# eridgd/WCT-TF

Measured on AMD Instinct MI355X. Metric: stylized frames/sec @512x512, 5-level relu5->1 pipeline, alpha=0.8, higher is better.
Workload: dtype f16

## Files before the change

### wct_tf_amd/csrc/api.hip

```cpp
#include "common.h"
#include "../../include/wct_hip.h"

#include <stdarg.h>
#include <stdio.h>
#include <string.h>
#include <stdlib.h>
#include <vector>
#include <cmath>
#include <algorithm>

static thread_local char g_err[512] = "";
void wct_set_error(const char* fmt, ...) {
  va_list ap;
  va_start(ap, fmt);
  vsnprintf(g_err, sizeof(g_err), fmt, ap);
  va_end(ap);
}
extern "C" const char* wct_last_error(void) { return g_err; }

struct DevBuf {
  void* p = nullptr;
  size_t cap = 0;
};

// ... 370 lines not shown
extern "C" int wct_set_encoder(wct_ctx* c, const float* pre_w, const float* pre_b,
                               const float* const* w, const float* const* b, int n_layers) {
  ARG_CHECK(c && pre_w && pre_b && w && b && n_layers == 13);
  HIP_TRY(hipSetDevice(c->device));
  std::vector<float> fw(27 * 64), fb(64);
  const float* w1 = w[0];
  for (int co = 0; co < 64; ++co) {
    double acc = b[0][co];
    for (int tap = 0; tap < 9; ++tap)
      for (int cp = 0; cp < 3; ++cp) acc += (double)pre_b[cp] * w1[(tap * 3 + cp) * 64 + co];
    fb[co] = (float)acc;
  }
  for (int tap = 0; tap < 9; ++tap)
    for (int ci = 0; ci < 3; ++ci)
      for (int co = 0; co < 64; ++co) {
        double acc = 0;
        for (int cp = 0; cp < 3; ++cp) acc += (double)pre_w[ci * 3 + cp] * w1[(tap * 3 + cp) * 64 + co];
        fw[(tap * 3 + ci) * 64 + co] = (float)acc;
      }
  if (c->first_w) { hipFree(c->first_w); c->first_w = nullptr; }
  if (c->first_b) { hipFree(c->first_b); c->first_b = nullptr; }
  std::vector<half_t> frag(2 * 2 * 2 * 64 * 8);
  for (int t = 0; t < 2; ++t)
    for (int ks = 0; ks < 2; ++ks)
      for (int l = 0; l < 64; ++l)
        for (int j = 0; j < 8; ++j) {
          const int co = t * 32 + (l & 31), k = ks * 16 + (l >> 5) * 8 + j;
          const float wv = k < 27 ? fw[k * 64 + co] : 0.f;
          const half_t hi = (half_t)wv;
          const half_t lo = (half_t)(wv - (float)hi);
          frag[((((t * 2 + ks) * 2 + 0) * 64) + l) * 8 + j] = hi;
          frag[((((t * 2 + ks) * 2 + 1) * 64) + l) * 8 + j] = lo;
        }
  TRY(upload(c, frag.data(), frag.size() * sizeof(half_t), (void**)&c->first_w));
  TRY(upload(c, fb.data(), fb.size() * sizeof(float), (void**)&c->first_b));
  if (c->first_w32) { hipFree(c->first_w32); c->first_w32 = nullptr; }
  TRY(upload(c, fw.data(), fw.size() * sizeof(float), (void**)&c->first_w32));
  for (int i = 0; i < 12; ++i) {
    TRY(pack_conv(c, w[i + 1], b[i + 1], ENC_CIN[i], ENC_COUT[i], &c->enc[i]));
    const int cin = ENC_CIN[i], cout = ENC_COUT[i];
    std::vector<float> wt((size_t)9 * cin * cout);
    for (int tap = 0; tap < 9; ++tap)
      for (int ci = 0; ci < cin; ++ci)
        for (int co = 0; co < cout; ++co) wt[((size_t)tap * cout + co) * cin + ci] = w[i + 1][((size_t)tap * cin + ci) * cout + co];
    if (c->enc_wt[i]) { hipFree(c->enc_wt[i]); c->enc_wt[i] = nullptr; }
    TRY(upload(c, wt.data(), wt.size() * sizeof(float), (void**)&c->enc_wt[i]));
  }
  c->enc_loaded = true;
  return WCT_OK;
}

static std::vector<PlanStep> decoder_plan(int level) {
  static const int arch5[] = {512, -1, 512, 512, 512, 0};
  static const int arch4[] = {256, -1, 256, 256, 256, 0};
  static const int arch3[] = {128, -1, 128, 0};
  static const int arch2[] = {64, -1, 0};
  static const int arch1[] = {64, 0};
  static const int* archs[6] = {nullptr, arch1, arch2, arch3, arch4, arch5};
  std::vector<PlanStep> plan;
  int cin = LEVEL_C[level];
  for (int d = level; d >= 1; --d)
    for (const int* a = archs[d]; *a != 0; ++a) {
      if (*a < 0) plan.push_back({'U', cin, cin, 0});
      else { plan.push_back({'C', cin, *a, 1}); cin = *a; }
    }
  plan.push_back({'C', cin, 3, 0});
  return plan;
}

extern "C" int wct_set_decoder(wct_ctx* c, int level, const float* const* w, const float* const* b, int n_layers) {
  ARG_CHECK(c && w && b && level >= 1 && level <= 5);
  HIP_TRY(hipSetDevice(c->device));
  Decoder& d = c->dec[level];
  free_decoder(d);
  d.plan = decoder_plan(level);
  int nconv = 0;
  for (auto& s : d.plan) nconv += s.kind == 'C';
  if (n_layers != nconv) {
    wct_set_error("decoder relu%d_1 needs %d conv layers, got %d", level, nconv, n_layers);
    return WCT_ERR_ARG;
  }
  int i = 0;
  for (auto& s : d.plan) {
    if (s.kind != 'C') continue;
    if (s.cout == 3) {
      std::vector<half_t> w16((size_t)4 * 64 * 8);
      for (int ks = 0; ks < 4; ++ks)
        for (int l = 0; l < 64; ++l)
          for (int j = 0; j < 8; ++j) {
            const int row = l & 31, cin = ks * 16 + (l >> 5) * 8 + j;
            const int tap = row / 3, co = row % 3;
            w16[((size_t)ks * 64 + l) * 8 + j] = row < 27 ? (half_t)w[i][((size_t)tap * 64 + cin) * 3 + co] : (half_t)0.f;
          }
      TRY(upload(c, w16.data(), w16.size() * sizeof(half_t), (void**)&d.last_w));
      TRY(upload(c, b[i], 3 * sizeof(float), (void**)&d.last_b));
    } else {
      d.convs.emplace_back();
      TRY(pack_conv(c, w[i], b[i], s.cin, s.cout, &d.convs.back()));
    }
    {
      float *w32 = nullptr, *b32 = nullptr;
      TRY(upload(c, w[i], (size_t)9 * s.cin * s.cout * sizeof(float), (void**)&w32));
      TRY(upload(c, b[i], (size_t)s.cout * sizeof(float), (void**)&b32));
      d.w32.push_back(w32); d.b32.push_back(b32); d.cin.push_back(s.cin); d.cout.push_back(s.cout);
    }
    ++i;
  }
  d.loaded = true;
  return WCT_OK;
}

static void level_dims(int H, int W, int level, int* h, int* w) {
  for (int l = 1; l < level; ++l) { H = (H + 1) / 2; W = (W + 1) / 2; }
  *h = H; *w = W;
}

static int check_min_size(const char* what, int H, int W, int level) {
  int h, w;
  level_dims(H, W, level, &h, &w);
  if (h < 2 || w < 2) {
    wct_set_error("%s %dx%d is too small for relu%d_1: its %dx%d feature map cannot be reflect-padded (need >= %dx%d pixels)",
                  what, H, W, level, h, w, (1 << (level - 1)) + 1, (1 << (level - 1)) + 1);
    return WCT_ERR_ARG;
  }
  return WCT_OK;
}


static int run_conv(wct_ctx* c, const ConvLayer& l, const half_t* x, half_t* y16, float* y32,
                    int B, int H, int W, int upsample, int relu, int pool = 0, float* usum = nullptr, unsigned* umax = nullptr,
                    bool tap_layer = false) {
  ConvArgs a;
  a.x = x; a.w = l.w; a.bias = l.b; a.y16 = y16; a.y32 = y32; a.usum = usum; a.umax = umax;
  a.w_wino = c->no_wino || tap_layer ? nullptr : l.ww;
  a.B = B; a.H = H; a.W = W; a.Cin = l.cin; a.Cout = l.cout; a.upsample = upsample; a.relu = relu; a.pool = pool;
  const double px = (double)B * H * W;
  const double in_px = upsample ? px / 4 : px;
  const double out_px = pool ? (double)B * ((H + 1) / 2) * ((W + 1) / 2) : px;
  ProfScope ps(c, conv3x3_wino_takes(a) ? 9 : 0, 2.0 * px * 9 * l.cin * l.cout,
               in_px * l.cin * 2 + out_px * l.cout * ((y16 ? 2 : 0) + (y32 ? 4 : 0)) + 9.0 * l.cin * l.cout * 2);
  return launch_conv3x3(a, c->stream);
}

static int run_encoder(wct_ctx* c, const float* img, int B, int H, int W, int clamp01, int deepest,
                       float* const taps32[6], float* const* usum = nullptr, unsigned* const* umax = nullptr) {
  if (!c->enc_loaded) { wct_set_error("encoder weights not set (wct_set_encoder)"); return WCT_ERR_STATE; }
  ARG_CHECK(deepest >= 1 && deepest <= 5 && H >= 2 && W >= 2);
  const size_t act_bytes = (size_t)B * H * W * 64 * sizeof(half_t);
  TRY(ensure(c, c->act[0], act_bytes));
  TRY(ensure(c, c->act[1], act_bytes));
  half_t* cur = (half_t*)c->act[0].p;
  half_t* nxt = (half_t*)c->act[1].p;
  static const int fuse_conv1_env = getenv("WCT_FUSE_CONV1") ? atoi(getenv("WCT_FUSE_CONV1")) : 1;
  const bool fuse_conv1 = fuse_conv1_env && deepest > 1 && !taps32[1];
  if (!fuse_conv1) {
    ConvFirstArgs a;
    a.x = img; a.wfrag = c->first_w; a.bias = c->first_b;
    a.y16 = deepest > 1 ? cur : nullptr; a.y32 = taps32[1];
    a.B = B; a.H = H; a.W = W; a.clamp01 = clamp01;
    a.usum = usum && taps32[1] ? usum[1] : nullptr; a.umax = a.usum ? umax[1] : nullptr;
    const double px = (double)B * H * W;
    ProfScope ps(c, 1, 2.0 * px * 27 * 64, px * (12 + 64 * ((a.y16 ? 2 : 0) + (a.y32 ? 4 : 0))));
    TRY(launch_conv_first(a, c->stream));
  }
  if (deepest == 1) return WCT_OK;
  static const int seq_tap[12] = {0, 2, 0, 3, 0, 0, 0, 4, 0, 0, 0, 5};
  static const int pool_after[12] = {1, 0, 1, 0, 0, 0, 1, 0, 0, 0, 1, 0};
  int h = H, w = W;
  for (int i = 0; i < 12; ++i) {
    const ConvLayer& l = c->enc[i];
    const int tap = seq_tap[i];
    const bool last = tap == deepest;
    const bool fuse = pool_after[i];
    float* const us = tap && taps32[tap] && usum ? usum[tap] : nullptr;
    if (i == 0 && fuse_conv1) {
      ConvArgs a;
      a.x = nullptr; a.w = l.w; a.bias = l.b; a.y16 = nxt; a.y32 = nullptr; a.usum = nullptr; a.umax = nullptr;
      a.B = B; a.H = h; a.W = w; a.Cin = 64; a.Cout = 64; a.upsample = 0; a.relu = 1; a.pool = fuse;
      a.img1 = img; a.w1frag = c->first_w; a.bias1 = c->first_b; a.clamp01 = clamp01;
      const double px = (double)B * h * w, out_px = fuse ? (double)B * ((h + 1) / 2) * ((w + 1) / 2) : px;
      ProfScope ps(c, 8, 2.0 * px * (27 * 64 + 9 * 64 * 64), px * 12 + out_px * 64 * 2 + 9.0 * 64 * 64 * 2);
      TRY(launch_conv3x3(a, c->stream));
    } else
    TRY(run_conv(c, l, cur, last ? nullptr : nxt, tap ? taps32[tap] : nullptr, B, h, w, 0, 1, fuse, us, us ? umax[tap] : nullptr, tap != 0));
    half_t* t = cur; cur = nxt; nxt = t;
    if (last) break;
    if (fuse) { h = (h + 1) / 2; w = (w + 1) / 2; }
  }
  return WCT_OK;
}

static int run_decoder(wct_ctx* c, int level, const half_t* feat16, int B, int h, int w, float* img_out) {
  Decoder& d = c->dec[level];
  if (!d.loaded) { wct_set_error("decoder weights for relu%d_1 not set (wct_set_decoder)", level); return WCT_ERR_STATE; }
  const int scale = 1 << (level - 1);
  const size_t act_bytes = (size_t)B * h * scale * w * scale * 64 * sizeof(half_t);
  const size_t deep_bytes = (size_t)B * h * w * LEVEL_C[level] * sizeof(half_t) * 4;
  TRY(ensure(c, c->act[0], act_bytes > deep_bytes ? act_bytes : deep_bytes));
  TRY(ensure(c, c->act[1], act_bytes > deep_bytes ? act_bytes : deep_bytes));
  const half_t* cur = feat16;
  half_t* bufs[2] = {(half_t*)c->act[0].p, (half_t*)c->act[1].p};
  int which = 0, ci = 0, up = 0;
  const size_t nsteps = d.plan.size();
  for (size_t si = 0; si < nsteps; ++si) {
    const PlanStep& s = d.plan[si];
    if (s.kind == 'U') { up = 1; h *= 2; w *= 2; continue; }
    if (s.cout == 3) {
      ARG_CHECK(up == 0);
      ConvLastArgs a;
      a.x = cur; a.wfrag = d.last_w; a.bias = d.last_b; a.y = img_out; a.B = B; a.H = h; a.W = w;
      const double px = (double)B * h * w;
      ProfScope ps(c, 2, 2.0 * px * 576 * 3, px * (128 + 12));
      TRY(launch_conv_last(a, c->stream));
    } else {
      half_t* out = bufs[which];
      TRY(run_conv(c, d.convs[ci++], cur, out, nullptr, B, h, w, up, 1));
      cur = out; which ^= 1; up = 0;
    }
  }
  return WCT_OK;
}

struct StageCost { double cov_flops, cov_bytes, apply_flops, apply_bytes, adain_bytes; };

template <typename Launch>
static int run_stages(wct_ctx* c, size_t ws_bytes, unsigned flags, const StageCost& cost, Launch&& launch) {
  TRY(ensure(c, c->wct_ws, ws_bytes));
  if (flags & WCT_FLAG_ADAIN) {
    ProfScope ps(c, 7, 0, cost.adain_bytes);
    return launch(0, 0);
  }
  const int mode = (flags & WCT_FLAG_MODE_NP) ? WCT_MODE_NP : WCT_MODE_TF;
  {
    ProfScope ps(c, 4, cost.cov_flops, cost.cov_bytes);
    TRY(launch(mode, WCT_STAGE_COV));
  }
  {
    ProfScope ps(c, 5, 0, 0);
    TRY(launch(mode, WCT_STAGE_EIG));
  }
  ProfScope ps(c, 6, cost.apply_flops, cost.apply_bytes);
  return launch(mode, WCT_STAGE_APPLY);
}

static int run_transform(wct_ctx* c, const float* fc, int Nc, const float* fs, int Ns, int C, int P,
                         float alpha, unsigned flags, float eps, half_t* out16, float* out32, int* sweeps_dev,
                         const WctFeatStats* st = nullptr, const WctStyleRef* prep = nullptr ,
                         const WctWarmRef* warm = nullptr ) {
  const int shared = (flags & WCT_FLAG_STYLE_SHARED) ? 1 : 0;
  const StageCost cost = {(double)P * 2.0 * C * C * ((double)Nc + Ns), (double)P * 2.0 * ((double)Nc + Ns) * C * 4,
                          (double)P * (2.0 * C * C * Nc + 6.0 * C * C * C), (double)P * Nc * C * (4 + (out16 ? 2 : 0) + (out32 ? 4 : 0)),
                          (double)P * (2.0 * Nc + 2.0 * Ns) * C * 4 + (double)P * Nc * C * 6};
  return run_stages(c, wct_workspace_bytes(C, Nc, Ns, P), flags, cost, [&](int mode, int stages) {
    if (!stages) return launch_adain(fc, Nc, fs, Ns, C, P, alpha, 1e-5f, out16, out32, c->wct_ws.p, c->wct_ws.cap, c->stream, shared, st, prep);
    return launch_wct(fc, Nc, fs, Ns, C, P, alpha, mode, eps, out16, out32, c->wct_ws.p, c->wct_ws.cap, sweeps_dev, stages, c->stream,
                      shared, c->eig_fail_dev, st, prep, warm);
  });
}

static int mix_weights(const float* weights, int K, float* lambda) {
  if (K < 1 || K > WCT_MIX_MAX) { wct_set_error("style mix: K = %d styles, must be 1 .. %d", K, (int)WCT_MIX_MAX); return WCT_ERR_ARG; }
  if (!weights) { wct_set_error("style mix: no weights"); return WCT_ERR_ARG; }
  double sum = 0.0;
  for (int k = 0; k < K; ++k) {
    if (!(weights[k] >= 0.f) || !std::isfinite(weights[k])) {
      wct_set_error("style mix: weight %d is %g; weights must be finite and >= 0", k, (double)weights[k]);
      return WCT_ERR_ARG;
    }
    sum += weights[k];
  }
  if (!(sum > 0.0) || !std::isfinite(sum)) { wct_set_error("style mix: the weights sum to %g, must be > 0", sum); return WCT_ERR_ARG; }
  for (int k = 0; k < K; ++k) lambda[k] = (float)(weights[k] / sum);
  return WCT_OK;
}

static int run_transform_mix(wct_ctx* c, const float* fc, int Nc, const float* const* fs, const int* Ns, int K, const float* lambda,
                             int C, float alpha, unsigned flags, float eps, half_t* out16, float* out32, int* sweeps_dev,
                             const WctFeatStats* st = nullptr, const WctStyleRef* prep = nullptr ) {
  double ns = 0;
  for (int k = 0; k < K; ++k) ns += Ns[k];
  const StageCost cost = {2.0 * C * C * (Nc + ns), 2.0 * (Nc + ns) * C * 4, 2.0 * C * C * Nc + 6.0 * C * C * C * (K + 1) + 2.0 * C * C * K,
                          (double)Nc * C * (4 + (out16 ? 2 : 0) + (out32 ? 4 : 0)), (2.0 * Nc + 2.0 * ns) * C * 4 + (double)Nc * C * 6};
  return run_stages(c, wct_mix_workspace_bytes(C, Nc, Ns, K, lambda), flags, cost, [&](int mode, int stages) {
    if (!stages) return launch_adain_mix(fc, Nc, fs, Ns, K, lambda, C, alpha, 1e-5f, out16, out32, c->wct_ws.p, c->wct_ws.cap, c->stream, st, prep);
    return launch_wct_mix(fc, Nc, fs, Ns, K, lambda, C, alpha, mode, eps, out16, out32, c->wct_ws.p, c->wct_ws.cap, sweeps_dev, stages,
                          c->stream, c->eig_fail_dev, st, prep);
  });
}

static int mask_check(const uint8_t* labels, size_t n, int K) {
  if (K < 1 || K > WCT_MIX_MAX) { wct_set_error("mask: K = %d styles, must be 1 .. %d", K, (int)WCT_MIX_MAX); return WCT_ERR_ARG; }
  uint8_t top = 0;
  for (size_t i = 0; i < n; ++i) top = labels[i] > top ? labels[i] : top;
  if (top >= K) { wct_set_error("mask: label %d with K = %d styles (labels must be 0 .. K - 1)", (int)top, K); return WCT_ERR_ARG; }
  return WCT_OK;
}

static void mask_counts(const uint8_t* mask, int Hm, int Wm, int h, int w, int stride, int K, int* nk) {
  for (int k = 0; k < K; ++k) nk[k] = 0;
  for (int i = 0; i < h; ++i) {
    const uint8_t* row = mask + (size_t)std::min(i * stride, Hm - 1) * Wm;
    for (int j = 0; j < w; ++j) ++nk[row[std::min(j * stride, Wm - 1)]];
  }
}

static int run_transform_masked(wct_ctx* c, const float* fc, int Nc, const MaskGeom& g, const int* nk, const float* const* fs,
                                const int* Ns, int K, int C, float alpha, unsigned flags, float eps, half_t* out16, float* out32,
                                int* sweeps_dev) {
  double ns = 0;
  int P = 0;
  for (int k = 0; k < K; ++k) { ns += nk[k] >= 2 ? Ns[k] : 0; P += nk[k] >= 2; }
  const StageCost cost = {2.0 * C * C * (Nc + ns), (4.0 * Nc + 2.0 * (Nc + ns)) * C * 4, 2.0 * C * C * Nc + 6.0 * C * C * C * P,
                          (double)Nc * C * (4 + (out16 ? 2 : 0) + (out32 ? 4 : 0)), (4.0 * Nc + 2.0 * ns) * C * 4 + (double)Nc * C * 6};
  return run_stages(c, wct_masked_workspace_bytes(C, Nc, nk, Ns, K), flags, cost, [&](int mode, int stages) {
    if (!stages) return launch_adain_masked(fc, Nc, g, nk, fs, Ns, K, C, alpha, 1e-5f, out16, out32, c->wct_ws.p, c->wct_ws.cap, c->stream);
    return launch_wct_masked(fc, Nc, g, nk, fs, Ns, K, C, alpha, mode, eps, out16, out32, c->wct_ws.p, c->wct_ws.cap, sweeps_dev, stages,
                             c->stream, c->eig_fail_dev);
  });
}

static int stage_in(wct_ctx* c, int slot, const void* host, size_t bytes, void** dev) {
  TRY(ensure(c, c->stage[slot], bytes));
  HIP_TRY(hipMemcpyAsync(c->stage[slot].p, host, bytes, hipMemcpyHostToDevice, c->stream));
  *dev = c->stage[slot].p;
  return WCT_OK;
}
static int fetch(wct_ctx* c, void* host, const void* dev, size_t bytes) {
  HIP_TRY(hipMemcpyAsync(host, dev, bytes, hipMemcpyDeviceToHost, c->stream));
  HIP_TRY(hipStreamSynchronize(c->stream));
  return WCT_OK;
}

extern "C" int wct_transform(wct_ctx* c, const float* content, int Nc, const float* style, int Ns, int C,
                             float alpha, int mode, float eps, float* out, int* sweeps_out) {
  ARG_CHECK(c && content && style && out && (mode == WCT_NP || mode == WCT_TF));
  HIP_TRY(hipSetDevice(c->device));
  TRY(eig_stale(c));
  void *dc, *ds;
  TRY(stage_in(c, 0, content, (size_t)Nc * C * 4, &dc));
  TRY(stage_in(c, 1, style, (size_t)Ns * C * 4, &ds));
  TRY(ensure(c, c->stage[2], (size_t)Nc * C * 4));
  TRY(ensure(c, c->stage[3], 256));
  TRY(run_transform(c, (float*)dc, Nc, (float*)ds, Ns, C, 1, alpha, mode == WCT_NP ? WCT_FLAG_MODE_NP : 0, eps,
                    nullptr, (float*)c->stage[2].p, (int*)c->stage[3].p));
  TRY(fetch(c, out, c->stage[2].p, (size_t)Nc * C * 4));
  if (sweeps_out) TRY(fetch(c, sweeps_out, c->stage[3].p, 2 * sizeof(int)));
  return eig_status(c);
}

extern "C" int wct_adain(wct_ctx* c, const float* content, int Nc, const float* style, int Ns, int C,
                         float alpha, float epsilon, float* out) {
  ARG_CHECK(c && content && style && out);
  HIP_TRY(hipSetDevice(c->device));
  void *dc, *ds;
  TRY(stage_in(c, 0, content, (size_t)Nc * C * 4, &dc));
  TRY(stage_in(c, 1, style, (size_t)Ns * C * 4, &ds));
  TRY(ensure(c, c->stage[2], (size_t)Nc * C * 4));
  TRY(ensure(c, c->wct_ws, wct_workspace_bytes(C, Nc, Ns, 1)));
  TRY(launch_adain((float*)dc, Nc, (float*)ds, Ns, C, 1, alpha, epsilon, nullptr, (float*)c->stage[2].p,
                   c->wct_ws.p, c->wct_ws.cap, c->stream, 0));
  return fetch(c, out, c->stage[2].p, (size_t)Nc * C * 4);
}

static int stage_in_multi(wct_ctx* c, const float* content, int Nc, const float* const* styles, const int* Ns, int K, int C,
                          void** dc, const float* ds[]) {
  TRY(stage_in(c, 0, content, (size_t)Nc * C * 4, dc));
  size_t total = 0;
  for (int k = 0; k < K; ++k) { ARG_CHECK(styles[k] && Ns[k] >= 1); total += (size_t)Ns[k] * C * 4; }
  TRY(ensure(c, c->mix_in, total));
  size_t off = 0;
  for (int k = 0; k < K; ++k) {
    char* d = (char*)c->mix_in.p + off;
    HIP_TRY(hipMemcpyAsync(d, styles[k], (size_t)Ns[k] * C * 4, hipMemcpyHostToDevice, c->stream));
    ds[k] = (const float*)d;
    off += (size_t)Ns[k] * C * 4;
  }
  TRY(ensure(c, c->stage[2], (size_t)Nc * C * 4));
  return ensure(c, c->stage[3], 2 * WCT_MIX_MAX * sizeof(int));
}

extern "C" int wct_transform_mix(wct_ctx* c, const float* content, int Nc, const float* const* styles, const int* Ns, int K,
                                 const float* weights, int C, float alpha, int mode, float eps, float* out, int* sweeps_out) {
  ARG_CHECK(c && content && styles && Ns && out && (mode == WCT_NP || mode == WCT_TF));
  float lambda[WCT_MIX_MAX];
  TRY(mix_weights(weights, K, lambda));
  HIP_TRY(hipSetDevice(c->device));
  TRY(eig_stale(c));
  void* dc;
  const float* ds[WCT_MIX_MAX];
  TRY(stage_in_multi(c, content, Nc, styles, Ns, K, C, &dc, ds));
  TRY(run_transform_mix(c, (float*)dc, Nc, ds, Ns, K, lambda, C, alpha, mode == WCT_NP ? WCT_FLAG_MODE_NP : 0, eps,
                        nullptr, (float*)c->stage[2].p, (int*)c->stage[3].p));
  TRY(fetch(c, out, c->stage[2].p, (size_t)Nc * C * 4));
  if (sweeps_out) {
    int sw[2 * WCT_MIX_MAX];
    TRY(fetch(c, sw, c->stage[3].p, 2 * K * sizeof(int)));
    sweeps_out[0] = sw[0];
    for (int k = 0; k < K; ++k) sweeps_out[1 + k] = sw[2 * k + 1];
  }
  return eig_status(c);
}

extern "C" int wct_adain_mix(wct_ctx* c, const float* content, int Nc, const float* const* styles, const int* Ns, int K,
                             const float* weights, int C, float alpha, float epsilon, float* out) {
// ... 242 lines not shown
  TRY(ensure(c, c->stage[1], (size_t)H * W * C * 2));
  TRY(ensure(c, c->stage[2], (size_t)Ho * Wo * C * 2));
  TRY(ensure(c, c->stage[3], (size_t)Ho * Wo * C * 4));
  TRY(launch_f32_to_f16((float*)dx, (half_t*)c->stage[1].p, (size_t)H * W * C, c->stream));
  TRY(launch_maxpool2x2((half_t*)c->stage[1].p, (half_t*)c->stage[2].p, 1, H, W, C, c->stream));
  TRY(launch_f16_to_f32((half_t*)c->stage[2].p, (float*)c->stage[3].p, (size_t)Ho * Wo * C, c->stream));
  return fetch(c, y, c->stage[3].p, (size_t)Ho * Wo * C * 4);
}

extern "C" int wct_encode(wct_ctx* c, const float* img01, int H, int W, int level, float* feat) {
  ARG_CHECK(c && img01 && feat && level >= 1 && level <= 5);
  HIP_TRY(hipSetDevice(c->device));
  TRY(check_min_size("image", H, W, level));
  int h, w;
  level_dims(H, W, level, &h, &w);
  void* dimg;
  TRY(stage_in(c, 0, img01, (size_t)H * W * 3 * 4, &dimg));
  const size_t fb = (size_t)h * w * LEVEL_C[level] * 4;
  TRY(ensure(c, c->feat_c, fb));
  float* taps[6] = {nullptr, nullptr, nullptr, nullptr, nullptr, nullptr};
  taps[level] = (float*)c->feat_c.p;
  TRY(run_encoder(c, (float*)dimg, 1, H, W, 0, level, taps));
  return fetch(c, feat, c->feat_c.p, fb);
}

extern "C" int wct_decode(wct_ctx* c, const float* feat, int h, int w, int level, float* img) {
  ARG_CHECK(c && feat && img && level >= 1 && level <= 5);
  HIP_TRY(hipSetDevice(c->device));
  const int C = LEVEL_C[level], scale = 1 << (level - 1);
  void* df;
  TRY(stage_in(c, 0, feat, (size_t)h * w * C * 4, &df));
  TRY(ensure(c, c->wct_out, (size_t)h * w * C * 2));
  TRY(launch_f32_to_f16((float*)df, (half_t*)c->wct_out.p, (size_t)h * w * C, c->stream));
  const size_t ib = (size_t)h * scale * w * scale * 3 * 4;
  TRY(ensure(c, c->img_t[0], ib));
  TRY(run_decoder(c, level, (half_t*)c->wct_out.p, 1, h, w, (float*)c->img_t[0].p));
  return fetch(c, img, c->img_t[0].p, ib);
}

extern "C" int wct_coral_stats(wct_ctx* c, const uint8_t* img, int H, int W, double sums[9]) {
  ARG_CHECK(c && img && sums && H > 0 && W > 0);
  HIP_TRY(hipSetDevice(c->device));
  const size_t npix = (size_t)H * W;
  void* dimg;
  TRY(stage_in(c, 0, img, npix * 3, &dimg));
  int nblocks = (int)((npix + 255) / 256);
  if (nblocks > 1024) nblocks = 1024;
  TRY(ensure(c, c->stage[1], (size_t)(nblocks + 1) * 9 * sizeof(unsigned long long)));
  unsigned long long* partial = (unsigned long long*)c->stage[1].p;
  unsigned long long* out9 = partial + (size_t)nblocks * 9;
  TRY(launch_coral_stats((uint8_t*)dimg, npix, partial, nblocks, out9, c->stream));
  unsigned long long host9[9];
  TRY(fetch(c, host9, out9, sizeof(host9)));
  for (int k = 0; k < 9; ++k) sums[k] = (double)host9[k];
  return WCT_OK;
}

extern "C" int wct_coral_apply(wct_ctx* c, const uint8_t* src, int H, int W, const double M[9],
                               const double src_mean[3], const double src_std[3], const double tgt_mean[3],
                               const double tgt_std[3], uint8_t* out_u8, double* out_f64) {
  ARG_CHECK(c && src && M && src_mean && src_std && tgt_mean && tgt_std && (out_u8 || out_f64) && H > 0 && W > 0);
  HIP_TRY(hipSetDevice(c->device));
  const size_t npix = (size_t)H * W;
  CoralApplyArgs a;
  for (int i = 0; i < 9; ++i) a.M[i] = M[i];
  for (int i = 0; i < 3; ++i) { a.src_mean[i] = src_mean[i]; a.src_std[i] = src_std[i]; a.tgt_mean[i] = tgt_mean[i]; a.tgt_std[i] = tgt_std[i]; }
  void* dsrc;
  TRY(stage_in(c, 0, src, npix * 3, &dsrc));
  if (out_u8) TRY(ensure(c, c->stage[1], npix * 3));
  if (out_f64) TRY(ensure(c, c->stage[2], npix * 3 * sizeof(double)));
  TRY(launch_coral_apply((uint8_t*)dsrc, npix, a, out_u8 ? (uint8_t*)c->stage[1].p : nullptr,
                         out_f64 ? (double*)c->stage[2].p : nullptr, c->stream));
  if (out_u8) TRY(fetch(c, out_u8, c->stage[1].p, npix * 3));
  if (out_f64) TRY(fetch(c, out_f64, c->stage[2].p, npix * 3 * sizeof(double)));
  return WCT_OK;
}

static int content_colors_checks(const void* stylized, int Ho, int Wo, const void* content, int Hc, int Wc, int B, const void* out) {
  if (!stylized || !content || !out) { wct_set_error("content colours: null image pointer"); return WCT_ERR_ARG; }
  if (B < 1 || B > 32) { wct_set_error("content colours: B = %d frames, must be 1 .. 32", B); return WCT_ERR_ARG; }
  if (Hc < 1 || Wc < 1 || Ho < Hc || Wo < Wc) {
    wct_set_error("content colours: a %dx%d stylized frame for a %dx%d content (the frame is never the smaller one)", Ho, Wo, Hc, Wc);
    return WCT_ERR_ARG;
  }
  return WCT_OK;
}

extern "C" int wct_content_colors_batch_dev(wct_ctx* c, const uint8_t* stylized, int Ho, int Wo, const uint8_t* content, int Hc,
                                            int Wc, int B, uint8_t* out) {
  ARG_CHECK(c != nullptr);
  TRY(content_colors_checks(stylized, Ho, Wo, content, Hc, Wc, B, out));
  HIP_TRY(hipSetDevice(c->device));
  ProfScope ps(c, 7, 0, (double)B * Ho * Wo * 3 * 2 + (double)B * Hc * Wc * 3);
  return launch_content_colors_u8(stylized, content, B, Ho, Wo, Hc, Wc, out, c->stream);
}

extern "C" int wct_content_colors(wct_ctx* c, const uint8_t* stylized, int Ho, int Wo, const uint8_t* content, int Hc, int Wc,
                                  uint8_t* out) {
  ARG_CHECK(c != nullptr);
  TRY(content_colors_checks(stylized, Ho, Wo, content, Hc, Wc, 1, out));
  HIP_TRY(hipSetDevice(c->device));
  void *ds, *dc;
  TRY(stage_in(c, 0, stylized, (size_t)Ho * Wo * 3, &ds));
  TRY(stage_in(c, 1, content, (size_t)Hc * Wc * 3, &dc));
  TRY(wct_content_colors_batch_dev(c, (uint8_t*)ds, Ho, Wo, (uint8_t*)dc, Hc, Wc, 1, (uint8_t*)ds));
  return fetch(c, out, ds, (size_t)Ho * Wo * 3);
}

extern "C" int wct_output_size(int Hc, int Wc, const int* levels, int n_levels, int* Ho, int* Wo) {
  ARG_CHECK(levels && Ho && Wo && n_levels >= 1 && Hc >= 2 && Wc >= 2);
  int H = Hc, W = Wc;
  for (int i = 0; i < n_levels; ++i) {
    ARG_CHECK(levels[i] >= 1 && levels[i] <= 5);
    TRY(check_min_size("content", H, W, levels[i]));
    int h, w;
    level_dims(H, W, levels[i], &h, &w);
    H = h << (levels[i] - 1); W = w << (levels[i] - 1);
  }
  *Ho = H; *Wo = W;
  return WCT_OK;
}

static int stylize_checks(wct_ctx* c, int Hc, int Wc, const uint8_t* const* styles, const int* Hs, const int* Ws, int K,
                          const int* levels, int n_levels, int* deepest, int* Ho, int* Wo) {
  *deepest = 0;
  for (int i = 0; i < n_levels; ++i) {
    ARG_CHECK(levels[i] >= 1 && levels[i] <= 5);
    if (levels[i] > *deepest) *deepest = levels[i];
    if (!c->dec[levels[i]].loaded) { wct_set_error("decoder weights for relu%d_1 not set", levels[i]); return WCT_ERR_STATE; }
  }
  TRY(wct_output_size(Hc, Wc, levels, n_levels, Ho, Wo));
  for (int k = 0; k < K; ++k) { ARG_CHECK(styles[k]); TRY(check_min_size("style", Hs[k], Ws[k], *deepest)); }
  return WCT_OK;
}

static int images_f32(wct_ctx* c, unsigned flags, const void* content, size_t nc, const void* style, size_t ns, const float** img_c,
                      const float** img_s) {
  *img_c = (const float*)content; *img_s = (const float*)style;
  if (flags & WCT_FLAG_IMAGES_F32) return WCT_OK;
  TRY(ensure(c, c->img_c, nc * 4));
  TRY(ensure(c, c->img_s, ns * 4));
  ProfScope ps(c, 7, 0, (double)(nc + ns) * 5);
  TRY(launch_u8_to_f32((const uint8_t*)content, (float*)c->img_c.p, nc, c->stream));
  TRY(launch_u8_to_f32((const uint8_t*)style, (float*)c->img_s.p, ns, c->stream));
  *img_c = (const float*)c->img_c.p; *img_s = (const float*)c->img_s.p;
  return WCT_OK;
}

static bool fuse_stats() {
  static const int on = getenv("WCT_FUSE_STATS") ? atoi(getenv("WCT_FUSE_STATS")) : 1;
  return on != 0;
}

template <typename StyleAt, typename Transform>
static int stylize_levels(wct_ctx* c, const float* img_c, const void* content_raw, int B, int Hc, int Wc, const int* levels,
                          int n_levels, unsigned flags, size_t umax_clear, int clear_from, StyleAt&& style_at,
                          Transform&& transform, uint8_t* out) {
  unsigned* const umax_c = (unsigned*)c->umax.p;
  const float* cur = img_c;
  int H = Hc, W = Wc;
  for (int i = 0; i < n_levels; ++i) {
    const int l = levels[i], C = LEVEL_C[l];
    int h, w;
    level_dims(H, W, l, &h, &w);
    TRY(ensure(c, c->feat_c, (size_t)B * h * w * C * 4));
    float* ctaps[6] = {nullptr, nullptr, nullptr, nullptr, nullptr, nullptr};
    ctaps[l] = (float*)c->feat_c.p;
    float* us_c[6] = {nullptr, nullptr, nullptr, nullptr, nullptr, nullptr};
    unsigned* um_c[6] = {nullptr, nullptr, nullptr, nullptr, nullptr, nullptr};
    if (fuse_stats() && w % 16 == 0) {
      TRY(ensure(c, c->usum_c, (size_t)B * h * (w / 16) * C * 4));
      us_c[l] = (float*)c->usum_c.p; um_c[l] = umax_c;
      if (i >= clear_from) HIP_TRY(hipMemsetAsync(umax_c, 0, umax_clear, c->stream));
    }
    WctFeatStats st = {};
    st.u[0] = us_c[l]; st.umax[0] = um_c[l];
    TRY(run_encoder(c, cur, B, H, W, i > 0, l, ctaps, us_c, um_c));
    TRY(ensure(c, c->wct_out, (size_t)B * h * w * C * 2));
    if (l == 5 && (flags & WCT_FLAG_SWAP5)) {
      int hs, ws;
      style_at(l, 0, &hs, &ws);
      ARG_CHECK(h >= c->ss_patch && w >= c->ss_patch && hs >= c->ss_patch && ws >= c->ss_patch);
      TRY(ensure(c, c->wct_ws, style_swap_workspace_bytes(C, h, w, hs, ws, c->ss_patch, c->ss_stride)));
      ProfScope ps(c, 7, 0, 0);
      for (int b = 0; b < B; ++b)
        TRY(launch_style_swap((float*)c->feat_c.p + (size_t)b * h * w * C, h, w, style_at(l, b, &hs, &ws), hs, ws, C, c->ss_alpha,
                              c->ss_patch, c->ss_stride, -1.f, (half_t*)c->wct_out.p + (size_t)b * h * w * C, nullptr,
                              c->wct_ws.p, c->wct_ws.cap, c->stream, c->eig_fail_dev));
    } else
      TRY(transform(i, l, C, h, w, st));
    const int scale = 1 << (l - 1);
    const int H2 = h * scale, W2 = w * scale;
    DevBuf& dst = c->img_t[i & 1];
    TRY(ensure(c, dst, (size_t)B * H2 * W2 * 3 * 4));
    TRY(run_decoder(c, l, (half_t*)c->wct_out.p, B, h, w, (float*)dst.p));
    cur = (float*)dst.p; H = H2; W = W2;
  }
  if (flags & WCT_FLAG_CONTENT_COLORS) {
    const int f32 = (flags & WCT_FLAG_IMAGES_F32) ? 1 : 0;
    ProfScope ps(c, 7, 0, (double)B * H * W * 3 * 5 + (double)B * Hc * Wc * 3 * (f32 ? 4 : 1));
    return launch_content_colors_f32(cur, content_raw, f32, B, H, W, Hc, Wc, out, c->stream);
  }
  ProfScope ps(c, 7, 0, (double)B * H * W * 3 * 5);
  return launch_f32_to_u8(cur, out, (size_t)B * H * W * 3, c->stream);
}

extern "C" int wct_stylize_batch_dev(wct_ctx* c, const uint8_t* content, int Hc, int Wc, const uint8_t* style,
                                     int Hs, int Ws, int B, const int* levels, int n_levels, float alpha,
                                     unsigned flags, uint8_t* out) {
  ARG_CHECK(c && content && style && out && levels && n_levels >= 1 && n_levels <= 16 && B >= 1 && B <= 32);
  HIP_TRY(hipSetDevice(c->device));
  int deepest, Ho, Wo;
  TRY(stylize_checks(c, Hc, Wc, &style, &Hs, &Ws, 1, levels, n_levels, &deepest, &Ho, &Wo));

  const int shared = (flags & WCT_FLAG_STYLE_SHARED) ? 1 : 0;
  const int Bs = shared ? 1 : B;
  const float *img_c, *img_s;
  TRY(images_f32(c, flags, content, (size_t)B * Hc * Wc * 3, style, (size_t)Bs * Hs * Ws * 3, &img_c, &img_s));
  const bool want_stats = fuse_stats();
  constexpr size_t UROW = 32 * UMAX_SLOTS;
  TRY(ensure(c, c->umax, 7 * UROW * sizeof(unsigned)));
  unsigned* const umax_c = (unsigned*)c->umax.p;
  if (want_stats) HIP_TRY(hipMemsetAsync(c->umax.p, 0, 7 * UROW * sizeof(unsigned), c->stream));
  float* taps[6] = {nullptr, nullptr, nullptr, nullptr, nullptr, nullptr};
  float* us_s[6] = {nullptr, nullptr, nullptr, nullptr, nullptr, nullptr};
  unsigned* um_s[6] = {nullptr, nullptr, nullptr, nullptr, nullptr, nullptr};
  for (int i = 0; i < n_levels; ++i) {
    const int l = levels[i];
    int h, w;
    level_dims(Hs, Ws, l, &h, &w);
    TRY(ensure(c, c->feat_s[l], (size_t)Bs * h * w * LEVEL_C[l] * 4));
    taps[l] = (float*)c->feat_s[l].p;
    if (want_stats && w % 16 == 0) {
      TRY(ensure(c, c->usum_s[l], (size_t)Bs * h * (w / 16) * LEVEL_C[l] * 4));
      us_s[l] = (float*)c->usum_s[l].p; um_s[l] = umax_c + UROW * l;
    }
  }
  TRY(run_encoder(c, img_s, Bs, Hs, Ws, 0, deepest, taps, us_s, um_s));

  auto style_at = [&](int l, int b, int* hs, int* ws) {
    level_dims(Hs, Ws, l, hs, ws);
    return (const float*)c->feat_s[l].p + (size_t)(shared ? 0 : b) * *hs * *ws * LEVEL_C[l];
  };
  return stylize_levels(c, img_c, content, B, Hc, Wc, levels, n_levels, flags, UROW * sizeof(unsigned), 1, style_at,
                        [&](int, int l, int C, int h, int w, WctFeatStats st) {
                          int hs, ws;
                          const float* fs = style_at(l, 0, &hs, &ws);
                          st.u[1] = us_s[l]; st.umax[1] = um_s[l];
                          return run_transform(c, (float*)c->feat_c.p, h * w, fs, hs * ws, C, B, alpha, flags, -1.f,
                                               (half_t*)c->wct_out.p, nullptr, nullptr, &st);
                        }, out);
}

extern "C" int wct_stylize(wct_ctx* c, const uint8_t* content, int Hc, int Wc, const uint8_t* style, int Hs, int Ws,
                           const int* levels, int n_levels, float alpha, unsigned flags, uint8_t* out) {
  ARG_CHECK(c && content && style && out);
  HIP_TRY(hipSetDevice(c->device));
  TRY(eig_stale(c));
  int Ho, Wo;
  TRY(wct_output_size(Hc, Wc, levels, n_levels, &Ho, &Wo));
  void *dc, *ds;
  const size_t px = (flags & WCT_FLAG_IMAGES_F32) ? sizeof(float) : 1;
  TRY(stage_in(c, 0, content, (size_t)Hc * Wc * 3 * px, &dc));
  TRY(stage_in(c, 1, style, (size_t)Hs * Ws * 3 * px, &ds));
  TRY(ensure(c, c->stage[2], (size_t)Ho * Wo * 3));
  TRY(wct_stylize_batch_dev(c, (uint8_t*)dc, Hc, Wc, (uint8_t*)ds, Hs, Ws, 1, levels, n_levels, alpha, flags,
                            (uint8_t*)c->stage[2].p));
  TRY(fetch(c, out, c->stage[2].p, (size_t)Ho * Wo * 3));
  return eig_status(c);
}

template <typename LevelTransform>
static int stylize_multi(wct_ctx* c, const uint8_t* content, int Hc, int Wc, const uint8_t* const* styles, const int* Hs,
                         const int* Ws, int K, const int* levels, int n_levels, unsigned flags, uint8_t* out,
                         LevelTransform&& level_transform) {
  HIP_TRY(hipSetDevice(c->device));
  int deepest, Ho, Wo;
  TRY(stylize_checks(c, Hc, Wc, styles, Hs, Ws, K, levels, n_levels, &deepest, &Ho, &Wo));
  TRY(eig_stale(c));
  const size_t px = (flags & WCT_FLAG_IMAGES_F32) ? sizeof(float) : 1;
  size_t ns_tot = 0, soff[WCT_MIX_MAX];
  for (int k = 0; k < K; ++k) { soff[k] = ns_tot; ns_tot += (size_t)Hs[k] * Ws[k] * 3; }
  const size_t nc = (size_t)Hc * Wc * 3;
  void* dc;
  TRY(stage_in(c, 0, content, nc * px, &dc));
  TRY(ensure(c, c->mix_in, ns_tot * px));
  for (int k = 0; k < K; ++k)
    HIP_TRY(hipMemcpyAsync((char*)c->mix_in.p + soff[k] * px, styles[k], (size_t)Hs[k] * Ws[k] * 3 * px, hipMemcpyHostToDevice, c->stream));
  const float *img_c, *img_s;
  TRY(images_f32(c, flags, dc, nc, c->mix_in.p, ns_tot, &img_c, &img_s));

  size_t foff[6][WCT_MIX_MAX];
  for (int i = 0; i < n_levels; ++i) {
    const int l = levels[i];
    size_t tot = 0;
    for (int k = 0; k < K; ++k) {
      int h, w;
      level_dims(Hs[k], Ws[k], l, &h, &w);
      foff[l][k] = tot;
      tot += (size_t)h * w * LEVEL_C[l];
    }
    TRY(ensure(c, c->feat_mix[l], tot * 4));
  }
  for (int k = 0; k < K; ++k) {
    float* taps[6] = {nullptr, nullptr, nullptr, nullptr, nullptr, nullptr};
    for (int i = 0; i < n_levels; ++i) taps[levels[i]] = (float*)c->feat_mix[levels[i]].p + foff[levels[i]][k];
    TRY(run_encoder(c, img_s + soff[k], 1, Hs[k], Ws[k], 0, deepest, taps));
  }

  TRY(ensure(c, c->umax, 32 * UMAX_SLOTS * sizeof(unsigned)));
  TRY(ensure(c, c->stage[2], (size_t)Ho * Wo * 3));
  auto style_at = [&](int l, int k, int* hs, int* ws) {
    level_dims(Hs[k], Ws[k], l, hs, ws);
    return (const float*)c->feat_mix[l].p + foff[l][k];
  };
  TRY(stylize_levels(c, img_c, dc, 1, Hc, Wc, levels, n_levels, flags, UMAX_SLOTS * sizeof(unsigned), 0, style_at,
                     [&](int i, int l, int C, int h, int w, const WctFeatStats& st) {
                       const float* fs[WCT_MIX_MAX];
                       int Ns[WCT_MIX_MAX];
                       for (int k = 0; k < K; ++k) {
                         int hs, ws;
                         fs[k] = style_at(l, k, &hs, &ws);
                         Ns[k] = hs * ws;
                       }
                       return level_transform(i, l, C, h, w, fs, Ns, &st);
                     }, (uint8_t*)c->stage[2].p));
  TRY(fetch(c, out, c->stage[2].p, (size_t)Ho * Wo * 3));
  return eig_status(c);
}

extern "C" int wct_stylize_mix(wct_ctx* c, const uint8_t* content, int Hc, int Wc, const uint8_t* const* styles, const int* Hs,
                               const int* Ws, int K, const float* weights, const int* levels, int n_levels, float alpha,
                               unsigned flags, uint8_t* out) {
  ARG_CHECK(c && content && styles && Hs && Ws && out && levels && n_levels >= 1 && n_levels <= 16);
  float lambda[WCT_MIX_MAX];
  TRY(mix_weights(weights, K, lambda));
  if ((flags & WCT_FLAG_SWAP5) && K > 1) {
    wct_set_error("style mix: WCT_FLAG_SWAP5 needs K = 1 (style-swap is not linear in the style; got K = %d)", K);
    return WCT_ERR_ARG;
  }
  if (flags & WCT_FLAG_STYLE_SHARED) { wct_set_error("style mix: WCT_FLAG_STYLE_SHARED is for wct_stylize_batch_dev"); return WCT_ERR_ARG; }
  return stylize_multi(c, content, Hc, Wc, styles, Hs, Ws, K, levels, n_levels, flags, out,
                       [&](int, int, int C, int h, int w, const float* const* fs, const int* Ns, const WctFeatStats* st) {
                         return run_transform_mix(c, (float*)c->feat_c.p, h * w, fs, Ns, K, lambda, C, alpha, flags, -1.f,
                                                  (half_t*)c->wct_out.p, nullptr, nullptr, st);
                       });
}

extern "C" int wct_stylize_masked(wct_ctx* c, const uint8_t* content, int Hc, int Wc, const uint8_t* mask, const uint8_t* const* styles,
                                  const int* Hs, const int* Ws, int K, const int* levels, int n_levels, float alpha, unsigned flags,
                                  uint8_t* out) {
  ARG_CHECK(c && content && mask && styles && Hs && Ws && out && levels && n_levels >= 1 && n_levels <= 16 && Hc >= 2 && Wc >= 2);
  TRY(mask_check(mask, (size_t)Hc * Wc, K));
  if ((flags & WCT_FLAG_SWAP5) && K > 1) {
    wct_set_error("mask: WCT_FLAG_SWAP5 needs K = 1 (style-swap is not a per-region affine map; got K = %d)", K);
    return WCT_ERR_ARG;
  }
  if (flags & WCT_FLAG_STYLE_SHARED) { wct_set_error("mask: WCT_FLAG_STYLE_SHARED is for wct_stylize_batch_dev"); return WCT_ERR_ARG; }
  std::vector<int> nk((size_t)n_levels * WCT_MIX_MAX);
  int H = Hc, W = Wc;
  for (int i = 0; i < n_levels; ++i) {
    ARG_CHECK(levels[i] >= 1 && levels[i] <= 5);
    int h, w;
    level_dims(H, W, levels[i], &h, &w);
    mask_counts(mask, Hc, Wc, h, w, 1 << (levels[i] - 1), K, &nk[(size_t)i * WCT_MIX_MAX]);
    H = h << (levels[i] - 1); W = w << (levels[i] - 1);
  }
  HIP_TRY(hipSetDevice(c->device));
  TRY(ensure(c, c->mask_in, (size_t)Hc * Wc));
  HIP_TRY(hipMemcpyAsync(c->mask_in.p, mask, (size_t)Hc * Wc, hipMemcpyHostToDevice, c->stream));
  return stylize_multi(c, content, Hc, Wc, styles, Hs, Ws, K, levels, n_levels, flags, out,
                       [&](int i, int l, int C, int h, int w, const float* const* fs, const int* Ns, const WctFeatStats*) {
                         const MaskGeom g = {(const uint8_t*)c->mask_in.p, Hc, Wc, w, 1 << (l - 1)};
                         return run_transform_masked(c, (float*)c->feat_c.p, h * w, g, &nk[(size_t)i * WCT_MIX_MAX], fs, Ns, K, C,
                                                     alpha, flags, -1.f, (half_t*)c->wct_out.p, nullptr, nullptr);
                       });
}

static int style_live(const wct_ctx* c, const wct_style* st) {
  if (st && std::find(c->styles.begin(), c->styles.end(), st) != c->styles.end()) return WCT_OK;
  wct_set_error("prepared style %p is not a live handle of this context (freed, or prepared by another context)", (const void*)st);
  return WCT_ERR_STATE;
}

static StyleState* state_find(wct_style* st, int level, const WctStyleKey& key, int kind) {
  for (auto& e : st->cache[level])
    if (e.kind == kind && e.key.nslab == key.nslab && e.key.nsplit == key.nsplit && e.key.ksplit == key.ksplit) return &e;
  return nullptr;
}

struct StyleNeed { int level; WctStyleKey key; int kind; };

static int style_fill(wct_ctx* c, wct_style* st, const std::vector<StyleNeed>& needs) {
  if (needs.empty()) return WCT_OK;
  HIP_TRY(hipStreamSynchronize(c->stream));
  int deepest = 0;
  float* taps[6] = {nullptr, nullptr, nullptr, nullptr, nullptr, nullptr};
  for (const StyleNeed& n : needs) {
    int h, w;
    level_dims(st->Hs, st->Ws, n.level, &h, &w);
    TRY(ensure(c, c->feat_s[n.level], (size_t)h * w * LEVEL_C[n.level] * 4));
    taps[n.level] = (float*)c->feat_s[n.level].p;
    deepest = std::max(deepest, n.level);
  }
// ... 760 lines not shown
```

### wct_tf_amd/csrc/common.h

```cpp
#pragma once
#include <hip/hip_runtime.h>
#include <stdint.h>
#include <stddef.h>

typedef _Float16 half_t;
typedef _Float16 half8 __attribute__((ext_vector_type(8)));
typedef _Float16 half4 __attribute__((ext_vector_type(4)));
typedef float f32x16 __attribute__((ext_vector_type(16)));
typedef float f32x4 __attribute__((ext_vector_type(4)));

#define WCT_OK 0
#define WCT_ERR_HIP -1
#define WCT_ERR_ARG -2
#define WCT_ERR_STATE -3
#define WCT_ERR_NOMEM -4
#define WCT_ERR_NOCONV -5

void wct_set_error(const char* fmt, ...);

#define HIP_TRY(expr)                                                          \
  do {                                                                         \
    hipError_t _e = (expr);                                                    \
    if (_e != hipSuccess) {                                                    \
      wct_set_error("%s failed: %s (%s:%d)", #expr, hipGetErrorString(_e),     \
                    __FILE__, __LINE__);                                       \
      return WCT_ERR_HIP;                                                      \
    }                                                                          \
  } while (0)

#define ARG_CHECK(cond)                                                        \
  do {                                                                         \
    if (!(cond)) {                                                             \
      wct_set_error("invalid argument: %s (%s:%d)", #cond, __FILE__, __LINE__);\
      return WCT_ERR_ARG;                                                      \
    }                                                                          \
  } while (0)

static inline int cdiv(int a, int b) { return (a + b - 1) / b; }


struct ConvArgs {
  const half_t* x;
  const half_t* w;
  const float* bias;
  half_t* y16;
  float* y32;
  int B, H, W;
  int Cin, Cout;
  int upsample;
  int relu;
  int pool;
  float* usum;
  unsigned* umax;
  const float* img1 = nullptr;
  const half_t* w1frag = nullptr;
  const float* bias1 = nullptr;
  int clamp01 = 0;
  const half_t* w_wino = nullptr;
};
constexpr int UMAX_SLOTS = 64;
__device__ __forceinline__ void umax_merge(unsigned* umax_img, int slot, float vmax, int lane) {
#pragma unroll
  for (int o = 32; o > 0; o >>= 1) vmax = fmaxf(vmax, __shfl_xor(vmax, o, 64));
  if (lane == 0) {
    unsigned* w = umax_img + (slot & (UMAX_SLOTS - 1));
    const unsigned bits = __builtin_bit_cast(unsigned, vmax);
    if (bits > __atomic_load_n(w, __ATOMIC_RELAXED)) atomicMax(w, bits);
  }
}
int launch_conv3x3(const ConvArgs& a, hipStream_t s);
bool conv3x3_wino_takes(const ConvArgs& a);
int launch_conv3x3_wino(const ConvArgs& a, hipStream_t s);

struct ConvFirstArgs {
  const float* x;
  const half_t* wfrag;
  const float* bias;
  half_t* y16;
  float* y32;
  int B, H, W;
  int clamp01;
  float* usum;
  unsigned* umax;
};

__device__ __forceinline__ void unit_row_sum4(f32x4& t) {
  float a = t[0], b = t[1], c = t[2], d = t[3];
#define WCT_DPP_STEP(ctrl)                                                             \
  "v_add_f32_dpp %0, %0, %0 " ctrl " row_mask:0xf bank_mask:0xf bound_ctrl:1\n"       \
  "v_add_f32_dpp %1, %1, %1 " ctrl " row_mask:0xf bank_mask:0xf bound_ctrl:1\n"       \
  "v_add_f32_dpp %2, %2, %2 " ctrl " row_mask:0xf bank_mask:0xf bound_ctrl:1\n"       \
  "v_add_f32_dpp %3, %3, %3 " ctrl " row_mask:0xf bank_mask:0xf bound_ctrl:1\n"
  asm volatile("s_nop 1\n"
               WCT_DPP_STEP("quad_perm:[1,0,3,2]")
               WCT_DPP_STEP("quad_perm:[2,3,0,1]")
               WCT_DPP_STEP("row_half_mirror")
               WCT_DPP_STEP("row_mirror")
               : "+v"(a), "+v"(b), "+v"(c), "+v"(d));
#undef WCT_DPP_STEP
  t[0] = a; t[1] = b; t[2] = c; t[3] = d;
}
int launch_conv_first(const ConvFirstArgs& a, hipStream_t s);

struct ConvLastArgs {
  const half_t* x;
  const half_t* wfrag;
  const float* bias;
  float* y;
  int B, H, W;
};
int launch_conv_last(const ConvLastArgs& a, hipStream_t s);

int launch_maxpool2x2(const half_t* x, half_t* y, int B, int H, int W, int C, hipStream_t s);
int launch_u8_to_f32(const uint8_t* x, float* y, size_t n, hipStream_t s);
int launch_f32_to_u8(const float* x, uint8_t* y, size_t n, hipStream_t s);
int launch_f32_to_f16(const float* x, half_t* y, size_t n, hipStream_t s);
int launch_f16_to_f32(const half_t* x, float* y, size_t n, hipStream_t s);

struct GemmArgs {
  const float* A; int lda; int a_kmajor;
  const float* B; int ldb; int b_kmajor;
  const float* a_sub_m;
  const float* b_sub_n;
  const float* a_sub_k;
  const float* a_scale_k;
  int M, N, K;
  int ksplit;
  float* out32; half_t* out16; int ldo;
  size_t out_split_stride;
  const float* bias_n;
  int nsplit;
  size_t sA, sB, s_sub_m, s_sub_n, s_sub_k, s_scale_k, s_out, s_bias;
  const float* A_odd;
  size_t sA_odd;
  int skip_shared;
  int blend; float alpha; unsigned* mabs;
  const float* mask_diag; size_t s_mask; int* mask_out; const int* mask_in;
};

int launch_gemm(GemmArgs g, int nsplit, int nbatch, hipStream_t s);

enum { WCT_MODE_NP = 0, WCT_MODE_TF = 1 };

struct WctFeatStats { const float* u[2]; const unsigned* umax[2]; };

struct WctStyleKey { int nslab, nsplit, ksplit; };
WctStyleKey wct_style_key(int C, int Nc, int Ns);
size_t wct_style_state_floats(int C);
size_t wct_style_workspace_bytes(int C, int Ns, const WctStyleKey& key);
int launch_style_state(const float* style, int Ns, int C, const WctStyleKey& key, int adain, int mode, float eps, void* workspace,
                       size_t workspace_bytes, int* eig_fail, hipStream_t s, float* state);
struct WctStyleRef { const float* state[8]; };
struct WctStyleSlots { const float* state[32]; };

struct WctWarmRef { float* basis; int valid; };

size_t wct_workspace_bytes(int C, int Nc, int Ns, int P);
int launch_wct(const float* content, int Nc, const float* style, int Ns, int C, int P,
               float alpha, int mode, float eps , half_t* out16, float* out32,
               void* workspace, size_t workspace_bytes, int* sweeps_dev, int stages, hipStream_t s,
               int shared_style ,
               int* eig_fail ,
               const struct WctFeatStats* stats = nullptr ,
               const struct WctStyleRef* prep = nullptr ,
               const struct WctWarmRef* warm = nullptr );
enum { WCT_STAGE_COV = 1, WCT_STAGE_EIG = 2, WCT_STAGE_APPLY = 4, WCT_STAGE_ALL = 7, WCT_STAGE_EIG_FP32UPDATE = 8 };
int launch_adain(const float* content, int Nc, const float* style, int Ns, int C, int P,
                 float alpha, float eps, half_t* out16, float* out32,
                 void* workspace, size_t workspace_bytes, hipStream_t s, int shared_style,
                 const struct WctFeatStats* stats = nullptr, const struct WctStyleRef* prep = nullptr);
enum { WCT_MIX_MAX = 8 };
size_t wct_mix_workspace_bytes(int C, int Nc, const int* Ns, int K, const float* lambda);
int launch_wct_mix(const float* content, int Nc, const float* const* styles, const int* Ns, int K, const float* lambda, int C,
                   float alpha, int mode, float eps, half_t* out16, float* out32, void* workspace, size_t workspace_bytes,
                   int* sweeps_dev, int stages, hipStream_t s, int* eig_fail, const struct WctFeatStats* stats = nullptr,
                   const struct WctStyleRef* prep = nullptr);
int launch_adain_mix(const float* content, int Nc, const float* const* styles, const int* Ns, int K, const float* lambda, int C,
                     float alpha, float eps, half_t* out16, float* out32, void* workspace, size_t workspace_bytes, hipStream_t s,
                     const struct WctFeatStats* stats = nullptr, const struct WctStyleRef* prep = nullptr);
struct MaskGeom { const uint8_t* mask; int Hm, Wm, w, stride; };
size_t mask_compact_workspace_bytes(int N, int G = 1);
int launch_mask_compact(const MaskGeom& g, int N, int K, int* perm, int* seg_off, void* workspace, hipStream_t s);
size_t wct_masked_workspace_bytes(int C, int Nc, const int* nk, const int* Ns, int K);
int launch_wct_masked(const float* content, int Nc, const MaskGeom& g, const int* nk, const float* const* styles, const int* Ns, int K,
                      int C, float alpha, int mode, float eps, half_t* out16, float* out32, void* workspace, size_t workspace_bytes,
                      int* sweeps_dev, int stages, hipStream_t s, int* eig_fail);
int launch_adain_masked(const float* content, int Nc, const MaskGeom& g, const int* nk, const float* const* styles, const int* Ns, int K,
                        int C, float alpha, float eps, half_t* out16, float* out32, void* workspace, size_t workspace_bytes, hipStream_t s);
size_t wct_masked_batch_workspace_bytes(int C, int Nc, int G, const int* nk, const int* Ns, int K);
int wct_masked_batch_pairs(int G, const int* nk, int K);
int launch_mask_compact_batch(const MaskGeom& g, int N, int K, int G, int* perm, int* seg_off, void* workspace, hipStream_t s);
int launch_wct_masked_batch(const float* content, int Nc, int G, const MaskGeom& g, const int* nk, const int* Ns, int K,
                            const WctStyleSlots& states, int C, float alpha, int mode, float eps, half_t* out16, float* out32,
                            void* workspace, size_t workspace_bytes, int stages, hipStream_t s, int* eig_fail);
int launch_adain_masked_batch(const float* content, int Nc, int G, const MaskGeom& g, const int* nk, const int* Ns, int K,
                              const WctStyleSlots& states, int C, float alpha, float eps, half_t* out16, float* out32,
                              void* workspace, size_t workspace_bytes, hipStream_t s);
int launch_jacobi_eigh(float* A, float* V, int C, int nmat, void* workspace,
                       size_t workspace_bytes, int* sweeps_done_dev, int* eig_fail, hipStream_t s);
size_t jacobi_workspace_bytes(int C, int nmat);

size_t style_swap_workspace_bytes(int C, int hc, int wc, int hs, int ws, int patch, int stride);
int launch_style_swap(const float* content, int hc, int wc, const float* style, int hs, int ws, int C,
                      float alpha, int patch, int stride, float eps, half_t* out16, float* out32,
                      void* workspace, size_t workspace_bytes, hipStream_t s, int* eig_fail);

int launch_im2col_act(const half_t* x, float* col, int B, int H, int W, int C, int upsample, hipStream_t s);
int launch_im2col_grad(const float* g, float* col, int B, int H, int W, int C, hipStream_t s);
int launch_reflect_fold(const float* gp, float* g, int B, int H, int W, int C, hipStream_t s);
int launch_relu_mask16(float* g, const half_t* act, size_t n, hipStream_t s);
int launch_relu_mask32(float* g, const float* act, size_t n, hipStream_t s);
int launch_upsample_adjoint(const float* gb, float* gs, int B, int h, int w, int C, hipStream_t s);
int launch_maxpool_adjoint(const half_t* pre, const float* gpool, float* gpre, int B, int H, int W, int C, hipStream_t s);
int launch_mse(const float* a, const float* b, size_t n, float weight, float* grad, int accumulate, double* partial,
               float* loss_out, hipStream_t s);
int launch_tv(const float* x, int B, int H, int W, int C, float weight, float* grad, double* partial, float* loss_out, hipStream_t s);
int launch_bias_grad(const float* g, size_t rows, int C, float* partial, float* out, hipStream_t s);
int launch_reduce_slabs(const float* partial, size_t n, int nslab, float* out, hipStream_t s);
int launch_adam(float* w, float* m, float* v, const float* g, size_t n, float lr_t, float b1, float b2, float eps, hipStream_t s);
int launch_pack_conv_frag(const float* w, half_t* frag, int cin, int cout, hipStream_t s);
int launch_pack_conv_wino_frag(const float* w, half_t* frag, int cin, int cout, hipStream_t s);
int launch_pack_last_frag(const float* w, half_t* frag, hipStream_t s);
int launch_transpose_w(const float* w, float* wt, int cin, int cout, int cout_pad, hipStream_t s);
int launch_pad3to4(const float* x, float* y, size_t n, hipStream_t s);
int launch_conv_dgrad(const float* g, const float* wt, int B, int H, int W, int cin, int cout,
                      float* col, float* gp, float* gin, void* scratch, hipStream_t s);
int launch_conv_wgrad(const half_t* x16, int upsample, const float* g, int ldg, int B, int H, int W, int cin, int cout,
                      float* col, float* partial, int nsplit, float* dw, void* scratch, hipStream_t s);
int conv_wgrad_splits(int B, int H, int W);
int launch_pow2_scale(const float* x, size_t n, void* scratch, hipStream_t s);
int launch_conv_first_dgrad(const float* g, const float* wf, float* gp, int B, int H, int W, hipStream_t s);

struct CoralApplyArgs {
  double M[9], src_mean[3], src_std[3], tgt_mean[3], tgt_std[3];
};
int launch_coral_stats(const uint8_t* img, size_t npix, unsigned long long* partial, int nblocks,
                       unsigned long long* out9, hipStream_t s);
int launch_coral_apply(const uint8_t* src, size_t npix, const CoralApplyArgs& a, uint8_t* out_u8,
                       double* out_f64, hipStream_t s);

int launch_content_colors_f32(const float* frame, const void* content, int content_f32, int B, int Ho, int Wo, int Hc, int Wc,
                              uint8_t* out, hipStream_t s);
int launch_content_colors_u8(const uint8_t* stylized, const uint8_t* content, int B, int Ho, int Wo, int Hc, int Wc, uint8_t* out,
                             hipStream_t s);
```

### wct_tf_amd/csrc/conv.hip

```cpp
#include "common.h"

typedef unsigned int u32x4 __attribute__((ext_vector_type(4)));
constexpr int TW = 16;
constexpr int PITCH = 20;
constexpr int BK = 32;

__device__ __forceinline__ int reflect_idx(int i, int n) {
  if (i < 0) i = -i;
  if (i >= n) i = 2 * n - 2 - i;
  i = i < 0 ? 0 : i;
  return i >= n ? n - 1 : i;
}

template <int MT, int NT, bool POOL, bool OUT32>
__device__ __forceinline__ void conv_epilogue_t(const ConvArgs& p, f32x16 (&acc)[NT][MT], int b, int y0, int x0, int n0,
                                                int wm, int wn, int lane, const unsigned char* bias_lds) {
  typedef _Float16 h2 __attribute__((ext_vector_type(2)));
  constexpr int OOB = (int)0x80000000u;
  const int frag_px = lane & 15;
  const int frag_py = (lane & 31) >> 4;
  const int kgrp = lane >> 5;
  const int Ho = POOL ? (p.H + 1) / 2 : p.H, Wo = POOL ? (p.W + 1) / 2 : p.W;
  const unsigned img_elems = (unsigned)Ho * Wo * p.Cout;
  const __amdgpu_buffer_rsrc_t r16 = __builtin_amdgcn_make_buffer_rsrc(
// ... 351 lines not shown
#pragma unroll
        for (int nt = 0; nt < NT; ++nt)
#pragma unroll
          for (int ks = 0; ks < 2; ++ks)
            wf[(t + 1) & 1][nt][ks] =
                __builtin_bit_cast(half8, __builtin_amdgcn_raw_buffer_load_b128(w_rsrc, wfrag[nt] + ks * 1024, wtap, 0));
      }
      if (!FUSE1 && tap == PF_TAP && more) load_patch(chunk_i + 1);
      read_group(bf[1], ky, kx, 1, buf);
      if (DB && tap == 8 && more) store_patch(buf ^ 1);
      __builtin_amdgcn_sched_barrier(0);
      mma_group(wf[t & 1], bf[0], 0);
      __builtin_amdgcn_sched_barrier(0);
      if (tap != 8) {
        read_group(bf[0], nky, nkx, 0, buf);
        __builtin_amdgcn_sched_barrier(0);
        mma_group(wf[t & 1], bf[1], 1);
      } else {
        mma_group(wf[t & 1], bf[1], 1);
        if (more) {
          __syncthreads();
          if (FUSE1) {
            make_patch(chunk_i + 1);
            __syncthreads();
          } else if (!DB) {
            if (PF_TAP > 8) load_patch(chunk_i + 1);
            store_patch(0);
            __syncthreads();
          }
        }
        read_group(bf[0], 0, 0, 0, DB ? buf ^ 1 : 0);
      }
      __builtin_amdgcn_sched_barrier(0);
    }
  }
  const bool more_tiles = FUSE1 && strip_i + 1 < strip && tx + strip_i + 1 < tiles_x;
  if (more_tiles) fetch_img(x0 + TW);
  conv_epilogue<MT, NT>(p, acc, b, y0, x0, n0, wm, wn, lane, smem + BIAS_OFF);
  if (more_tiles) {
    ++strip_i;
    x0 += TW;
    goto next_tile;
  }
}

template <int TH, int BN, int WM, int WN, bool FUSE1 = false>
static int launch_conv_cfg(const ConvArgs& a, hipStream_t s) {
  const int tiles_x = cdiv(a.W, TW), tiles_y = cdiv(a.H, TH);
  const int n_tiles = a.Cout / BN;
  constexpr int PH = TH + 2;
  constexpr int NBUF = ((TH / 2) / WM) * ((BN / 32) / WN) > 8 ? 2 : 1;
  const size_t lds = (size_t)NBUF * (PH * PITCH * 64 + 4096) + BN * sizeof(float)
                     + (FUSE1 ? (size_t)(TH + 4) * 20 * 3 * 4 + 64 + 8192 + 256 + 9 * 1024 : 0);
  const long tiles = (long)tiles_x * tiles_y * a.B;
  const int strip = !FUSE1 ? 1 : tiles >= 8192 ? 4 : tiles >= 4096 ? 2 : 1;
  dim3 grid((FUSE1 ? cdiv(tiles_x, strip) : tiles_x) * tiles_y * n_tiles, a.B);
  if (lds > 64 * 1024) {
    static bool raised[16] = {};
    int dev = 0;
    HIP_TRY(hipGetDevice(&dev));
    if (dev >= 0 && dev < 16 && !raised[dev]) {
      HIP_TRY(hipFuncSetAttribute(reinterpret_cast<const void*>(&conv3x3_mfma_kernel<TH, BN, WM, WN, FUSE1>),
                                  hipFuncAttributeMaxDynamicSharedMemorySize, (int)lds));
      raised[dev] = true;
    }
  }
  hipLaunchKernelGGL((conv3x3_mfma_kernel<TH, BN, WM, WN, FUSE1>), grid, dim3(256), lds, s, a, tiles_x, tiles_y, n_tiles, strip);
  HIP_TRY(hipGetLastError());
  return WCT_OK;
}

int launch_conv3x3(const ConvArgs& a, hipStream_t s) {
  ARG_CHECK(a.Cin % 64 == 0 && a.Cout % 64 == 0 && a.H > 1 && a.W > 1 && a.B > 0);
  ARG_CHECK(!a.upsample || (a.H % 2 == 0 && a.W % 2 == 0));
  ARG_CHECK((size_t)a.H * a.W * a.Cin * 2 < ((size_t)1 << 31));
  ARG_CHECK((size_t)a.H * a.W * a.Cout * (a.y32 ? 4 : 2) < ((size_t)1 << 31));
  ARG_CHECK(!a.usum || (a.y32 && a.umax && a.relu && a.W % 16 == 0));
  ARG_CHECK(!a.pool || (a.relu && !a.y32));
  if (conv3x3_wino_takes(a)) return launch_conv3x3_wino(a, s);
  if (a.img1) {
    ARG_CHECK(a.Cin == 64 && a.Cout == 64 && !a.upsample && a.w1frag && a.bias1);
    return launch_conv_cfg<32, 64, 4, 1, true>(a, s);
  }
  const long px16 = (long)cdiv(a.W, TW) * cdiv(a.H, 16) * a.B;
  const long px32 = (long)cdiv(a.W, TW) * cdiv(a.H, 32) * a.B;
  if (a.Cout % 128 == 0 && px16 * (a.Cout / 128) >= 512) return launch_conv_cfg<16, 128, 2, 2>(a, s);
  if (px32 * (a.Cout / 64) >= 512) return launch_conv_cfg<32, 64, 4, 1>(a, s);
  if (a.Cout % 128 == 0 && px16 * (a.Cout / 128) >= 256) return launch_conv_cfg<16, 128, 2, 2>(a, s);
  if (px16 * (a.Cout / 64) >= 256) return launch_conv_cfg<16, 64, 4, 1>(a, s);
  return launch_conv_cfg<8, 64, 2, 2>(a, s);
}

__global__ __launch_bounds__(256) void conv_first_kernel(ConvFirstArgs p, int strips_x) {
  constexpr int CF_TILES = 4, PATCH_N = 18 * 18 * 3, PER = (PATCH_N + 255) / 256;
  __shared__ float patch[PATCH_N + 4];
  __shared__ __attribute__((aligned(16))) unsigned char tr[4][32 * 256];
  typedef unsigned int u32x4 __attribute__((ext_vector_type(4)));
  const int tid = threadIdx.x, lane = tid & 63, wave = tid >> 6;
  const int sx = blockIdx.x % strips_x, ty = blockIdx.x / strips_x;
  const int b = blockIdx.y;
  const int y0 = ty * 16;
  const float* xb = p.x + (size_t)b * p.H * p.W * 3;
  int e_row[PER], e_px[PER], e_c[PER];
#pragma unroll
  for (int i = 0; i < PER; ++i) {
    const int e = tid + i * 256;
    const int pix = e < PATCH_N ? e / 3 : 0;
    e_c[i] = e < PATCH_N ? e - pix * 3 : 0;
    const int py = pix / 18;
    e_px[i] = pix - py * 18;
    e_row[i] = reflect_idx(y0 - 1 + py, p.H) * p.W;
  }
  float pre[PER];
  auto fetch = [&](int x0) {
#pragma unroll
    for (int i = 0; i < PER; ++i) {
      float v = xb[((size_t)e_row[i] + reflect_idx(x0 - 1 + e_px[i], p.W)) * 3 + e_c[i]];
      pre[i] = p.clamp01 ? fminf(fmaxf(v, 0.f), 1.f) : v;
    }
  };
  auto park = [&]() {
#pragma unroll
    for (int i = 0; i < PER; ++i) if (tid + i * 256 < PATCH_N) patch[tid + i * 256] = pre[i];
  };
  if (tid < 4) patch[PATCH_N + tid] = 0.f;
  fetch(sx * CF_TILES * 16);
  half8 wh[2][2], wl[2][2];
#pragma unroll
  for (int t = 0; t < 2; ++t)
#pragma unroll
    for (int ks = 0; ks < 2; ++ks) {
      wh[t][ks] = *reinterpret_cast<const half8*>(p.wfrag + (((t * 2 + ks) * 2 + 0) * 64 + lane) * 8);
      wl[t][ks] = *reinterpret_cast<const half8*>(p.wfrag + (((t * 2 + ks) * 2 + 1) * 64 + lane) * 8);
    }
  const int frag_px = lane & 15, frag_py = (lane & 31) >> 4, kgrp = lane >> 5;
  int addr[2][8];
#pragma unroll
  for (int ks = 0; ks < 2; ++ks)
#pragma unroll
    for (int j = 0; j < 8; ++j) {
      const int k = ks * 16 + kgrp * 8 + j;
      const int ky = k / 9, kp = k - ky * 9;
      addr[ks][j] = k < 27 ? (((wave * 4 + frag_py + ky) * 18 + frag_px) * 3 + kp) * 4 : 972 * 4;
    }
  f32x4 bias[2][4];
#pragma unroll
  for (int nt = 0; nt < 2; ++nt)
#pragma unroll
    for (int rq = 0; rq < 4; ++rq) bias[nt][rq] = *reinterpret_cast<const f32x4*>(p.bias + nt * 32 + 8 * rq + 4 * kgrp);
  park();
  __syncthreads();
  const unsigned char* pb = reinterpret_cast<const unsigned char*>(patch);
  unsigned char* const wt = tr[wave];
  float vmax = 0.f;
  for (int tile = 0; tile < CF_TILES; ++tile) {
  const int x0 = (sx * CF_TILES + tile) * 16;
  if (x0 >= p.W) break;
  const bool next = tile + 1 < CF_TILES && x0 + 16 < p.W;
  if (next) fetch(x0 + 16);
#pragma unroll
  for (int mt = 0; mt < 2; ++mt) {
    f32x16 acc[2];
#pragma unroll
    for (int nt = 0; nt < 2; ++nt)
#pragma unroll
      for (int r = 0; r < 16; ++r) acc[nt][r] = 0.f;
#pragma unroll
    for (int ks = 0; ks < 2; ++ks) {
      half8 bh, bl;
#pragma unroll
      for (int j = 0; j < 8; ++j) {
        const int off = (ks * 16 + kgrp * 8 + j < 27) ? mt * 2 * 54 * 4 : 0;
        const float v = *reinterpret_cast<const float*>(pb + addr[ks][j] + off);
        bh[j] = (half_t)v;
        bl[j] = (half_t)(v - (float)bh[j]);
      }
#pragma unroll
      for (int nt = 0; nt < 2; ++nt) {
        acc[nt] = __builtin_amdgcn_mfma_f32_32x32x16_f16(wl[nt][ks], bh, acc[nt], 0, 0, 0);
        acc[nt] = __builtin_amdgcn_mfma_f32_32x32x16_f16(wh[nt][ks], bl, acc[nt], 0, 0, 0);
        acc[nt] = __builtin_amdgcn_mfma_f32_32x32x16_f16(wh[nt][ks], bh, acc[nt], 0, 0, 0);
      }
    }
    const int px = lane & 31;
#pragma unroll
    for (int nt = 0; nt < 2; ++nt)
#pragma unroll
      for (int rq = 0; rq < 4; ++rq) {
        f32x4 v;
#pragma unroll
        for (int j = 0; j < 4; ++j) v[j] = fmaxf(acc[nt][rq * 4 + j] + bias[nt][rq][j], 0.f);
        const int piece = nt * 8 + 2 * rq + kgrp;
        *reinterpret_cast<f32x4*>(wt + (px * 16 + (piece ^ (px & 15))) * 16) = v;
        if (p.usum) {
          f32x4 t = v;
          unit_row_sum4(t);
          const int sy = y0 + wave * 4 + mt * 2 + frag_py;
          if (sy < p.H) {
            vmax = fmaxf(fmaxf(vmax, fmaxf(v[0], v[1])), fmaxf(v[2], v[3]));
            if (frag_px == 0)
              *reinterpret_cast<f32x4*>(p.usum + ((size_t)b * (p.H * (p.W >> 4)) + sy * (p.W >> 4) + (x0 >> 4)) * 64 + piece * 4) = t;
          }
        }
      }
    __builtin_amdgcn_fence(__ATOMIC_RELEASE, "wavefront");
    __builtin_amdgcn_wave_barrier();
    const int oy0 = y0 + wave * 4 + mt * 2;
    if (p.y32) {
      const int piece = lane & 15;
#pragma unroll
      for (int it = 0; it < 8; ++it) {
        const int q = it * 4 + (lane >> 4);
        const int oy = oy0 + (q >> 4), ox = x0 + (q & 15);
        const f32x4 v = *reinterpret_cast<const f32x4*>(wt + (q * 16 + (piece ^ (q & 15))) * 16);
        if (oy < p.H && ox < p.W) *reinterpret_cast<f32x4*>(p.y32 + (((size_t)b * p.H + oy) * p.W + ox) * 64 + piece * 4) = v;
      }
    }
    if (p.y16) {
      const int c8 = lane & 7;
#pragma unroll
      for (int it = 0; it < 4; ++it) {
        const int q = it * 8 + (lane >> 3);
        const int oy = oy0 + (q >> 4), ox = x0 + (q & 15);
        const f32x4 v0 = *reinterpret_cast<const f32x4*>(wt + (q * 16 + ((2 * c8) ^ (q & 15))) * 16);
        const f32x4 v1 = *reinterpret_cast<const f32x4*>(wt + (q * 16 + ((2 * c8 + 1) ^ (q & 15))) * 16);
        half8 h;
#pragma unroll
        for (int j = 0; j < 4; ++j) { h[j] = (half_t)v0[j]; h[4 + j] = (half_t)v1[j]; }
        if (oy < p.H && ox < p.W) *reinterpret_cast<half8*>(p.y16 + (((size_t)b * p.H + oy) * p.W + ox) * 64 + c8 * 8) = h;
      }
    }
    __builtin_amdgcn_fence(__ATOMIC_RELEASE, "wavefront");
    __builtin_amdgcn_wave_barrier();
  }
  if (next) {
    __syncthreads();
    park();
    __syncthreads();
  }
  }
  if (p.usum) umax_merge(p.umax + b * UMAX_SLOTS, (int)blockIdx.x * 4 + wave, vmax, lane);
}

int launch_conv_first(const ConvFirstArgs& a, hipStream_t s) {
  ARG_CHECK(a.H > 1 && a.W > 1 && a.B > 0);
  ARG_CHECK(!a.usum || (a.y32 && a.umax && a.W % 16 == 0));
  const int strips_x = cdiv(a.W, 64), tiles_y = cdiv(a.H, 16);
  hipLaunchKernelGGL(conv_first_kernel, dim3(strips_x * tiles_y, a.B), dim3(256), 0, s, a, strips_x);
  HIP_TRY(hipGetLastError());
  return WCT_OK;
}

__global__ __launch_bounds__(256) void conv_last_kernel(ConvLastArgs p, int tiles_x) {
  constexpr int PP = 33;
  __shared__ float part[18 * 18 * PP];
  const int tid = threadIdx.x, lane = tid & 63, wave = tid >> 6;
  const int tx = blockIdx.x % tiles_x, ty = blockIdx.x / tiles_x;
  const int b = blockIdx.y;
  const int y0 = ty * 16, x0 = tx * 16;
  const half_t* xb = p.x + (size_t)b * p.H * p.W * 64;
  half8 wf[4];
#pragma unroll
  for (int ks = 0; ks < 4; ++ks) wf[ks] = *reinterpret_cast<const half8*>(p.wfrag + (ks * 64 + lane) * 8);
  half8 bf[3][4];
  int qs[3];
#pragma unroll
  for (int i = 0; i < 3; ++i) {
    const int tile = wave + 4 * i;
    const int q = tile * 32 + (lane & 31);
    qs[i] = q;
    const int qq = q < 324 ? q : 323;
    const int py = qq / 18, px = qq - py * 18;
    const int iy = reflect_idx(y0 - 1 + py, p.H), ix = reflect_idx(x0 - 1 + px, p.W);
    const half_t* src = xb + ((size_t)iy * p.W + ix) * 64 + (lane >> 5) * 8;
    if (tile < 11) {
#pragma unroll
      for (int ks = 0; ks < 4; ++ks) bf[i][ks] = *reinterpret_cast<const half8*>(src + ks * 16);
    }
  }
#pragma unroll
  for (int i = 0; i < 3; ++i) {
    if (wave + 4 * i >= 11) break;
    f32x16 acc;
#pragma unroll
    for (int r = 0; r < 16; ++r) acc[r] = 0.f;
#pragma unroll
    for (int ks = 0; ks < 4; ++ks) acc = __builtin_amdgcn_mfma_f32_32x32x16_f16(wf[ks], bf[i][ks], acc, 0, 0, 0);
    if (qs[i] < 324) {
#pragma unroll
      for (int r = 0; r < 16; ++r)
        part[qs[i] * PP + (r & 3) + 8 * (r >> 2) + 4 * (lane >> 5)] = acc[r];
    }
  }
  __syncthreads();
  const int ly = tid >> 4, lx = tid & 15;
  const int oy = y0 + ly, ox = x0 + lx;
  float a0 = p.bias[0], a1 = p.bias[1], a2 = p.bias[2];
#pragma unroll
  for (int tap = 0; tap < 9; ++tap) {
    const int ky = tap / 3, kx = tap - ky * 3;
    const float* pq = part + ((ly + ky) * 18 + lx + kx) * PP + tap * 3;
    a0 += pq[0]; a1 += pq[1]; a2 += pq[2];
  }
  if (oy < p.H && ox < p.W) {
    float* o = p.y + (((size_t)b * p.H + oy) * p.W + ox) * 3;
    o[0] = a0; o[1] = a1; o[2] = a2;
  }
}

int launch_conv_last(const ConvLastArgs& a, hipStream_t s) {
  ARG_CHECK(a.H > 1 && a.W > 1 && a.B > 0);
  const int tiles_x = cdiv(a.W, 16), tiles_y = cdiv(a.H, 16);
  hipLaunchKernelGGL(conv_last_kernel, dim3(tiles_x * tiles_y, a.B), dim3(256), 0, s, a, tiles_x);
  HIP_TRY(hipGetLastError());
  return WCT_OK;
}

__global__ void maxpool_kernel(const half_t* x, half_t* y, int B, int H, int W, int C, int Ho, int Wo) {
  const int c8 = C / 8;
  size_t total = (size_t)B * Ho * Wo * c8;
  for (size_t i = blockIdx.x * (size_t)blockDim.x + threadIdx.x; i < total; i += (size_t)gridDim.x * blockDim.x) {
    int c = (int)(i % c8);
    size_t t = i / c8;
    int ox = (int)(t % Wo); t /= Wo;
    int oy = (int)(t % Ho);
    int b = (int)(t / Ho);
    const half_t* xb = x + (size_t)b * H * W * C;
    int iy = oy * 2, ix = ox * 2;
    half8 m = *reinterpret_cast<const half8*>(xb + ((size_t)iy * W + ix) * C + c * 8);
    if (ix + 1 < W) m = __builtin_elementwise_max(m, *reinterpret_cast<const half8*>(xb + ((size_t)iy * W + ix + 1) * C + c * 8));
    if (iy + 1 < H) {
      m = __builtin_elementwise_max(m, *reinterpret_cast<const half8*>(xb + ((size_t)(iy + 1) * W + ix) * C + c * 8));
      if (ix + 1 < W) m = __builtin_elementwise_max(m, *reinterpret_cast<const half8*>(xb + ((size_t)(iy + 1) * W + ix + 1) * C + c * 8));
    }
    *reinterpret_cast<half8*>(y + i * 8) = m;
  }
}

int launch_maxpool2x2(const half_t* x, half_t* y, int B, int H, int W, int C, hipStream_t s) {
  ARG_CHECK(C % 8 == 0);
  const int Ho = (H + 1) / 2, Wo = (W + 1) / 2;
  size_t total = (size_t)B * Ho * Wo * (C / 8);
  int blocks = (int)((total + 255) / 256);
  if (blocks > 4096) blocks = 4096;
  hipLaunchKernelGGL(maxpool_kernel, dim3(blocks), dim3(256), 0, s, x, y, B, H, W, C, Ho, Wo);
  HIP_TRY(hipGetLastError());
  return WCT_OK;
}

__global__ void u8_to_f32_kernel(const uint8_t* x, float* y, size_t n) {
  for (size_t i = blockIdx.x * (size_t)blockDim.x + threadIdx.x; i < n; i += (size_t)gridDim.x * blockDim.x)
    y[i] = (float)((double)x[i] / 255.0);
}
__global__ void f32_to_u8_kernel(const float* x, uint8_t* y, size_t n) {
  for (size_t i = blockIdx.x * (size_t)blockDim.x + threadIdx.x; i < n; i += (size_t)gridDim.x * blockDim.x) {
    float v = fminf(fmaxf(x[i], 0.f), 1.f) * 255.f;
    y[i] = (uint8_t)v;
  }
}
__global__ void f32_to_f16_kernel(const float* x, half_t* y, size_t n) {
  for (size_t i = blockIdx.x * (size_t)blockDim.x + threadIdx.x; i < n; i += (size_t)gridDim.x * blockDim.x) y[i] = (half_t)x[i];
}
__global__ void f16_to_f32_kernel(const half_t* x, float* y, size_t n) {
  for (size_t i = blockIdx.x * (size_t)blockDim.x + threadIdx.x; i < n; i += (size_t)gridDim.x * blockDim.x) y[i] = (float)x[i];
}

static inline int ew_blocks(size_t n) {
  size_t b = (n + 255) / 256;
  return (int)(b > 4096 ? 4096 : (b ? b : 1));
}
int launch_u8_to_f32(const uint8_t* x, float* y, size_t n, hipStream_t s) {
  hipLaunchKernelGGL(u8_to_f32_kernel, dim3(ew_blocks(n)), dim3(256), 0, s, x, y, n);
  HIP_TRY(hipGetLastError());
  return WCT_OK;
}
int launch_f32_to_u8(const float* x, uint8_t* y, size_t n, hipStream_t s) {
  hipLaunchKernelGGL(f32_to_u8_kernel, dim3(ew_blocks(n)), dim3(256), 0, s, x, y, n);
  HIP_TRY(hipGetLastError());
  return WCT_OK;
}
int launch_f32_to_f16(const float* x, half_t* y, size_t n, hipStream_t s) {
  hipLaunchKernelGGL(f32_to_f16_kernel, dim3(ew_blocks(n)), dim3(256), 0, s, x, y, n);
  HIP_TRY(hipGetLastError());
  return WCT_OK;
}
int launch_f16_to_f32(const half_t* x, float* y, size_t n, hipStream_t s) {
  hipLaunchKernelGGL(f16_to_f32_kernel, dim3(ew_blocks(n)), dim3(256), 0, s, x, y, n);
  HIP_TRY(hipGetLastError());
  return WCT_OK;
}
```

### wct_tf_amd/csrc/stats_gemm.hip

```cpp
#include "wct_stages.h"


struct StatArgs {
  const float* x[2];
  int n[2];
  const float* u[2];
  const unsigned* umax[2];
  const float* mean;
  float* partial;
  float* absmax;
  int C, nslab;
  int shared_style;
};

__global__ __launch_bounds__(256) void colsum_kernel(StatArgs p) {
  __shared__ f32x4 red[256];
  const int mat = blockIdx.y, slab = blockIdx.x;
  if (skip_style_mat(mat, p.shared_style)) return;
  const int b = mat & 1, pair = mat >> 1;
  const int C = p.C, cq = C / 4;
  const int nrp = 256 / cq;
  const int tid = threadIdx.x;
  const int rp = tid / cq, c4 = tid % cq;
  const int N = p.n[b];
// ... 134 lines not shown
      }
    }
  }
};

constexpr float REFRESH_RATIO = 1e-4f;
__device__ __forceinline__ bool refresh_needed(const float* Am, int C, int tid) {
  float dmax = 0.f, dmin = 3.0e38f;
  for (int i = tid; i < C; i += 256) {
    const float d = Am[(size_t)i * C + i];
    dmax = fmaxf(dmax, fabsf(d));
    if (d > 3.3e-6f) dmin = fminf(dmin, d);
  }
  for (int o = 32; o > 0; o >>= 1) { dmax = fmaxf(dmax, __shfl_xor(dmax, o, 64)); dmin = fminf(dmin, __shfl_xor(dmin, o, 64)); }
  __shared__ float red[2][4];
  if ((tid & 63) == 0) { red[0][tid >> 6] = dmax; red[1][tid >> 6] = dmin; }
  __syncthreads();
  dmax = fmaxf(fmaxf(red[0][0], red[0][1]), fmaxf(red[0][2], red[0][3]));
  dmin = fminf(fminf(red[1][0], red[1][1]), fminf(red[1][2], red[1][3]));
  return dmin < 3.0e38f && dmin < REFRESH_RATIO * dmax;
}

template <int BM, int BN>
__global__ __launch_bounds__(256, 4) void gemm_f32_kernel(GemmArgs p) {
  constexpr int TM = BM / 64, TN = BN / 64;
  constexpr int PA = BM + 4, PB = BN + 4;
  __shared__ __attribute__((aligned(16))) float As[GK * PA];
  __shared__ __attribute__((aligned(16))) float Bs[GK * PB];
  const int tid = threadIdx.x, lane = tid & 63, wave = tid >> 6;
  const int wm = wave >> 1, wn = wave & 1;
  const int m0 = blockIdx.y * BM, n0 = blockIdx.x * BN;
  const int batch = blockIdx.z / p.nsplit, split = blockIdx.z % p.nsplit;
  if (p.skip_shared && skip_style_mat(batch, p.skip_shared)) return;
  if (p.mask_in && !p.mask_in[batch]) return;
  if (p.mask_diag) {
    const bool need = refresh_needed(p.mask_diag + batch * p.s_mask, p.M, tid);
    if (p.mask_out && blockIdx.x == 0 && blockIdx.y == 0 && split == 0 && tid == 0) p.mask_out[batch] = need ? 1 : 0;
    if (!need) return;
  }
  const int kbeg = split * p.ksplit;
  const int kend = min(p.K, kbeg + p.ksplit);
  if (p.A_odd) p.A = (batch & 1) ? p.A_odd + (batch >> 1) * p.sA_odd : p.A + (batch >> 1) * p.sA;
  else p.A += batch * p.sA;
  p.B += batch * p.sB;
  if (p.a_sub_m) p.a_sub_m += batch * p.s_sub_m;
  if (p.b_sub_n) p.b_sub_n += batch * p.s_sub_n;
  if (p.a_sub_k) p.a_sub_k += batch * p.s_sub_k;
  if (p.a_scale_k) p.a_scale_k += batch * p.s_scale_k;
  if (p.bias_n) p.bias_n += batch * p.s_bias;

  f32x16 acc[TM][TN];
#pragma unroll
  for (int i = 0; i < TM; ++i)
#pragma unroll
    for (int j = 0; j < TN; ++j)
#pragma unroll
      for (int r = 0; r < 16; ++r) acc[i][j][r] = 0.f;

  GemmStage<BM> sa;
  GemmStage<BN> sb;
  if (kbeg < kend) {
    sa.load(p.A, p.lda, p.a_kmajor, kbeg, kend, m0, p.M, p.a_sub_m, p.a_sub_k, p.a_scale_k, tid);
    sb.load(p.B, p.ldb, p.b_kmajor, kbeg, kend, n0, p.N, p.b_sub_n, nullptr, nullptr, tid);
  }
  for (int k0 = kbeg; k0 < kend; k0 += GK) {
    sa.store(As, p.a_kmajor, tid);
    sb.store(Bs, p.b_kmajor, tid);
    __syncthreads();
    if (k0 + GK < kend) {
      sa.load(p.A, p.lda, p.a_kmajor, k0 + GK, kend, m0, p.M, p.a_sub_m, p.a_sub_k, p.a_scale_k, tid);
      sb.load(p.B, p.ldb, p.b_kmajor, k0 + GK, kend, n0, p.N, p.b_sub_n, nullptr, nullptr, tid);
    }
#pragma unroll
    for (int kk = 0; kk < GK; kk += 2) {
      float a[TM], b[TN];
      const int kr = kk + (lane >> 5);
#pragma unroll
      for (int i = 0; i < TM; ++i) a[i] = As[kr * PA + (wm * TM + i) * 32 + (lane & 31)];
#pragma unroll
      for (int j = 0; j < TN; ++j) b[j] = Bs[kr * PB + (wn * TN + j) * 32 + (lane & 31)];
#pragma unroll
      for (int i = 0; i < TM; ++i)
#pragma unroll
        for (int j = 0; j < TN; ++j)
          acc[i][j] = __builtin_amdgcn_mfma_f32_32x32x2f32(a[i], b[j], acc[i][j], 0, 0, 0);
    }
    __syncthreads();
  }

  float* o32 = p.out32 ? p.out32 + batch * p.s_out + (size_t)split * p.out_split_stride : nullptr;
  half_t* o16 = p.out16 ? p.out16 + batch * p.s_out : nullptr;
  float biasv[TN];
#pragma unroll
  for (int j = 0; j < TN; ++j) {
    const int gn = n0 + (wn * TN + j) * 32 + (lane & 31);
    biasv[j] = (p.bias_n && gn < p.N) ? p.bias_n[gn] : 0.f;
  }
#pragma unroll
  for (int j = 0; j < TN; ++j) asm volatile("" : "+v"(biasv[j]));
  float av = 0.f;
#pragma unroll
  for (int i = 0; i < TM; ++i)
#pragma unroll
    for (int j = 0; j < TN; ++j) {
      const int gn = n0 + (wn * TN + j) * 32 + (lane & 31);
      const float bias = biasv[j];
#pragma unroll
      for (int r = 0; r < 16; ++r) {
        const int gm = m0 + (wm * TM + i) * 32 + (r & 3) + 8 * (r >> 2) + 4 * (lane >> 5);
        if (gm < p.M && gn < p.N) {
          float v = acc[i][j][r] + bias;
          if (p.blend) {
            v = p.alpha * acc[i][j][r];
            if (gm == gn) v += 1.f - p.alpha;
            av = fmaxf(av, fabsf(v));
          }
          if (o32) o32[(size_t)gm * p.ldo + gn] = v;
          if (o16) o16[(size_t)gm * p.ldo + gn] = (half_t)v;
        }
      }
    }
  if (p.blend) {
    for (int o = 32; o > 0; o >>= 1) av = fmaxf(av, __shfl_xor(av, o, 64));
    if (lane == 0 && av < 1e30f) atomicMax(p.mabs + batch, __float_as_uint(av));
  }
}

int launch_gemm(GemmArgs g, int nsplit, int nbatch, hipStream_t s) {
  g.nsplit = nsplit;
  const int gz = nsplit * nbatch;
  const bool small_grid = (long)cdiv(g.M, 128) * cdiv(g.N, 128) * gz < 256;
  if (g.M >= 128 && g.N >= 128 && !small_grid) {
    dim3 grid(cdiv(g.N, 128), cdiv(g.M, 128), gz);
    hipLaunchKernelGGL((gemm_f32_kernel<128, 128>), grid, dim3(256), 0, s, g);
  } else if (g.M >= 128 && !small_grid) {
    dim3 grid(cdiv(g.N, 64), cdiv(g.M, 128), gz);
    hipLaunchKernelGGL((gemm_f32_kernel<128, 64>), grid, dim3(256), 0, s, g);
  } else {
    dim3 grid(cdiv(g.N, 64), cdiv(g.M, 64), gz);
    hipLaunchKernelGGL((gemm_f32_kernel<64, 64>), grid, dim3(256), 0, s, g);
  }
  HIP_TRY(hipGetLastError());
  return WCT_OK;
}

struct CovArgs {
  const float* x[2];
  int n[2];
  const float* mean;
  const float* scale;
  float* partial;
  int C, ksplit, nsplit, ntile;
  int shared_style;
};

template <int BT>
__global__ __launch_bounds__(256, 2) void cov_f16x2_kernel(CovArgs p) {
  constexpr int TM = BT / 64;
  constexpr int KPT = BT * 32 / 256;
  constexpr int NPC = KPT / 8;
  __shared__ __attribute__((aligned(16))) unsigned char lds[4][BT * 64];
  const int tid = threadIdx.x, lane = tid & 63, wave = tid >> 6;
  const int wm = wave >> 1, wn = wave & 1;
  int ti = 0, rem = blockIdx.x;
  while (rem >= p.ntile - ti) { rem -= p.ntile - ti; ++ti; }
  const int tj = ti + rem;
  const bool diag = ti == tj;
  const int m0 = ti * BT, n0 = tj * BT;
  const int mat = blockIdx.z, split = blockIdx.y;
  if (skip_style_mat(mat, p.shared_style)) return;
  const int side = mat & 1, pair = mat >> 1;
  const int N = p.n[side], C = p.C;
  const float* x = p.x[side] + (size_t)pair * N * C;
  const int kbeg = split * p.ksplit;
  const int kend = min(N, kbeg + p.ksplit);
  const float sc = p.scale[mat];

  const int c = tid % BT;
  const int kg = __builtin_amdgcn_readfirstlane(tid / BT);
  const float mean_a = p.mean[mat * C + min(m0 + c, C - 1)];
  const float mean_b = p.mean[mat * C + min(n0 + c, C - 1)];
  const __amdgpu_buffer_rsrc_t rsrc = __builtin_amdgcn_make_buffer_rsrc((void*)x, 0, (int)((size_t)N * C * 4), 0x00020000);
  const int voff_a = min(m0 + c, C - 1) * 4, voff_b = min(n0 + c, C - 1) * 4;

  f32x16 acc[TM][TM];
#pragma unroll
  for (int i = 0; i < TM; ++i)
#pragma unroll
    for (int j = 0; j < TM; ++j)
#pragma unroll
      for (int r = 0; r < 16; ++r) acc[i][j][r] = 0.f;

  auto load = [&](float (&r)[KPT], int voff, int k0) {
#pragma unroll
    for (int j = 0; j < KPT; ++j)
      r[j] = __builtin_bit_cast(float, __builtin_amdgcn_raw_buffer_load_b32(rsrc, voff, (k0 + kg * KPT + j) * C * 4, 0));
  };
  auto split_store = [&](const float (&r)[KPT], float mean, int k0, bool tail, unsigned char* hi, unsigned char* lo) {
#pragma unroll
    for (int q = 0; q < NPC; ++q) {
      half8 h, l;
#pragma unroll
      for (int j = 0; j < 8; ++j) {
        const float s_in = (!tail || k0 + kg * KPT + q * 8 + j < kend) ? sc : 0.f;
        const float v = (r[q * 8 + j] - mean) * s_in;
        h[j] = (half_t)v;
        l[j] = (half_t)(v - (float)h[j]);
      }
      const int chunk = kg * NPC + q;
      const int off = (c * 4 + (chunk ^ ((c >> 2) & 3))) * 16;
      *reinterpret_cast<half8*>(hi + off) = h;
      *reinterpret_cast<half8*>(lo + off) = l;
    }
  };
  auto mma_stage = [&](const unsigned char* bh, const unsigned char* bl) {
#pragma unroll
    for (int ks = 0; ks < 2; ++ks) {
      const int chunk = ks * 2 + (lane >> 5);
      half8 ah[TM], al[TM], bhf[TM], blf[TM];
#pragma unroll
      for (int i = 0; i < TM; ++i) {
        const int r = (wm * TM + i) * 32 + (lane & 31);
        const int off = (r * 4 + (chunk ^ ((r >> 2) & 3))) * 16;
        ah[i] = *reinterpret_cast<const half8*>(lds[0] + off);
        al[i] = *reinterpret_cast<const half8*>(lds[1] + off);
      }
#pragma unroll
      for (int j = 0; j < TM; ++j) {
        const int r = (wn * TM + j) * 32 + (lane & 31);
        const int off = (r * 4 + (chunk ^ ((r >> 2) & 3))) * 16;
        bhf[j] = *reinterpret_cast<const half8*>(bh + off);
        blf[j] = *reinterpret_cast<const half8*>(bl + off);
      }
#pragma unroll
      for (int i = 0; i < TM; ++i)
#pragma unroll
        for (int j = 0; j < TM; ++j) {
          acc[i][j] = __builtin_amdgcn_mfma_f32_32x32x16_f16(al[i], bhf[j], acc[i][j], 0, 0, 0);
          acc[i][j] = __builtin_amdgcn_mfma_f32_32x32x16_f16(ah[i], blf[j], acc[i][j], 0, 0, 0);
          acc[i][j] = __builtin_amdgcn_mfma_f32_32x32x16_f16(ah[i], bhf[j], acc[i][j], 0, 0, 0);
        }
    }
  };

  float ra[KPT], rb[KPT];
  if (diag) {
    if (kbeg < kend) load(ra, voff_a, kbeg);
    for (int k0 = kbeg; k0 < kend; k0 += 32) {
      if (k0 + 32 <= kend) split_store(ra, mean_a, k0, false, lds[0], lds[1]);
      else split_store(ra, mean_a, k0, true, lds[0], lds[1]);
      __syncthreads();
      if (k0 + 32 < kend) load(ra, voff_a, k0 + 32);
      mma_stage(lds[0], lds[1]);
      __syncthreads();
    }
  } else {
    if (kbeg < kend) { load(ra, voff_a, kbeg); load(rb, voff_b, kbeg); }
    for (int k0 = kbeg; k0 < kend; k0 += 32) {
      if (k0 + 32 <= kend) {
        split_store(ra, mean_a, k0, false, lds[0], lds[1]);
        split_store(rb, mean_b, k0, false, lds[2], lds[3]);
      } else {
        split_store(ra, mean_a, k0, true, lds[0], lds[1]);
        split_store(rb, mean_b, k0, true, lds[2], lds[3]);
      }
      __syncthreads();
      if (k0 + 32 < kend) { load(ra, voff_a, k0 + 32); load(rb, voff_b, k0 + 32); }
      mma_stage(lds[2], lds[3]);
      __syncthreads();
    }
  }

  float* out = p.partial + ((size_t)mat * p.nsplit + split) * C * C;
#pragma unroll
  for (int i = 0; i < TM; ++i)
#pragma unroll
    for (int j = 0; j < TM; ++j) {
      const int gn = n0 + (wn * TM + j) * 32 + (lane & 31);
#pragma unroll
      for (int r = 0; r < 16; ++r) {
        const int gm = m0 + (wm * TM + i) * 32 + (r & 3) + 8 * (r >> 2) + 4 * (lane >> 5);
        if (gm < C && gn < C) out[(size_t)gm * C + gn] = acc[i][j][r];
      }
    }
}

__global__ __launch_bounds__(256) void cov_finish_kernel(const float* partial, const float* scale, float* cov, int C, int nsplit, int BT,
                                                         float inv0, float inv1, float eps, int shared_style, float* cov0 = nullptr) {
  __shared__ float tt[64][65];
  const int mat = blockIdx.z;
  if (skip_style_mat(mat, shared_style)) return;
  const size_t cc = (size_t)C * C;
  const int r0 = blockIdx.y * 64, c0 = blockIdx.x * 64, tid = threadIdx.x, ty = tid >> 4, tx = tid & 15;
  const bool mirror = r0 / BT > c0 / BT;
  const float* pb = partial + (size_t)mat * nsplit * cc;
  const float sc = scale[mat];
  const float f = ((mat & 1) == 0 ? inv0 : inv1) / (sc * sc);
  f32x4 acc[4];
#pragma unroll
  for (int i = 0; i < 4; ++i) {
    const int r = (mirror ? c0 : r0) + ty * 4 + i, c = (mirror ? r0 : c0) + tx * 4;
    f32x4 sum = {0.f, 0.f, 0.f, 0.f};
    if (r < C && c < C)
      for (int k = 0; k < nsplit; ++k) sum += *reinterpret_cast<const f32x4*>(pb + (size_t)k * cc + (size_t)r * C + c);
    acc[i] = sum;
  }
  if (mirror) {
#pragma unroll
    for (int i = 0; i < 4; ++i)
#pragma unroll
      for (int j = 0; j < 4; ++j) tt[ty * 4 + i][tx * 4 + j] = acc[i][j];
    __syncthreads();
#pragma unroll
    for (int i = 0; i < 4; ++i)
#pragma unroll
      for (int j = 0; j < 4; ++j) acc[i][j] = tt[tx * 4 + j][ty * 4 + i];
  }
#pragma unroll
  for (int i = 0; i < 4; ++i) {
    const int r = r0 + ty * 4 + i, c = c0 + tx * 4;
    if (r >= C || c >= C) continue;
    f32x4 v = acc[i] * f;
#pragma unroll
    for (int j = 0; j < 4; ++j) if (r == c + j) v[j] += eps;
    *reinterpret_cast<f32x4*>(cov + (size_t)mat * cc + (size_t)r * C + c) = v;
    if (cov0) *reinterpret_cast<f32x4*>(cov0 + (size_t)mat * cc + (size_t)r * C + c) = v;
  }
}

int launch_means(const float* content, int Nc, const float* style, int Ns, int C, int P,
                        const WctCarve& w, bool with_var, int shared_style, hipStream_t s, const WctFeatStats* fs) {
  StatArgs sa;
  sa.x[0] = content; sa.x[1] = style; sa.n[0] = Nc; sa.n[1] = Ns;
  for (int b = 0; b < 2; ++b) {
    sa.u[b] = fs && fs->umax[b] ? fs->u[b] : nullptr;
    sa.umax[b] = sa.u[b] ? fs->umax[b] : nullptr;
  }
  sa.mean = nullptr; sa.partial = w.stat_partial; sa.absmax = w.absmax; sa.C = C; sa.nslab = w.nslab; sa.shared_style = shared_style;
  hipLaunchKernelGGL(colsum_kernel, dim3(w.nslab, 2 * P), dim3(256), 0, s, sa);
  hipLaunchKernelGGL(colsum_finish_kernel, dim3(cdiv(C, 256), 2 * P), dim3(256), 0, s, w.stat_partial, w.mean, C, w.nslab, (float)Nc, (float)Ns, shared_style,
                     (const float*)w.absmax, w.scale);
  if (with_var) {
    sa.mean = w.mean; sa.absmax = nullptr;
    hipLaunchKernelGGL(colsum_kernel, dim3(w.nslab, 2 * P), dim3(256), 0, s, sa);
    hipLaunchKernelGGL(colsum_finish_kernel, dim3(cdiv(C, 256), 2 * P), dim3(256), 0, s, w.stat_partial, w.var, C, w.nslab, (float)Nc, (float)Ns, shared_style,
                       (const float*)nullptr, (float*)nullptr);
  }
  HIP_TRY(hipGetLastError());
  return WCT_OK;
}

int launch_cov(const float* content, int Nc, const float* style, int Ns, int C, int P, const WctCarve& w, float eps, int shared_style,
               hipStream_t s) {
  const int BT = C >= 128 ? 128 : 64;
  {
    CovArgs ca;
    ca.x[0] = content; ca.x[1] = style; ca.n[0] = Nc; ca.n[1] = Ns;
    ca.mean = w.mean; ca.scale = w.scale; ca.partial = w.cov_partial;
    ca.C = C; ca.ksplit = w.ksplit; ca.nsplit = w.nsplit; ca.ntile = cdiv(C, BT); ca.shared_style = shared_style;
    dim3 grid(ca.ntile * (ca.ntile + 1) / 2, w.nsplit, 2 * P);
    if (BT == 128) hipLaunchKernelGGL((cov_f16x2_kernel<128>), grid, dim3(256), 0, s, ca);
    else hipLaunchKernelGGL((cov_f16x2_kernel<64>), grid, dim3(256), 0, s, ca);
    HIP_TRY(hipGetLastError());
  }
  hipLaunchKernelGGL(cov_finish_kernel, dim3(cdiv(C, 64), cdiv(C, 64), 2 * P), dim3(256), 0, s, w.cov_partial, w.scale, w.A, C,
                     w.nsplit, BT, 1.f / (float)(Nc - 1), 1.f / (float)(Ns - 1), eps, shared_style, w.A0);
  HIP_TRY(hipGetLastError());
  return WCT_OK;
}

static int launch_slot_means(const float* x, int N, int C, int m, int nslab, const WctCarve& w, bool with_var, hipStream_t s,
                             const float* u = nullptr, const unsigned* umax = nullptr) {
  StatArgs sa = {};
  sa.x[0] = sa.x[1] = x; sa.n[0] = sa.n[1] = N;
  sa.u[0] = umax ? u : nullptr; sa.umax[0] = sa.u[0] ? umax : nullptr;
  float* partial = w.stat_partial + (size_t)m * w.nslab * C;
  float* absmax = w.absmax + (size_t)m * w.nslab;
  sa.mean = nullptr; sa.partial = partial; sa.absmax = absmax; sa.C = C; sa.nslab = nslab; sa.shared_style = 0;
  hipLaunchKernelGGL(colsum_kernel, dim3(nslab, 1), dim3(256), 0, s, sa);
  hipLaunchKernelGGL(colsum_finish_kernel, dim3(cdiv(C, 256), 1), dim3(256), 0, s, partial, w.mean + (size_t)m * C, C, nslab, (float)N,
                     (float)N, 0, (const float*)absmax, w.scale + m);
  if (with_var) {
    sa.mean = w.mean + (size_t)m * C; sa.absmax = nullptr;
    hipLaunchKernelGGL(colsum_kernel, dim3(nslab, 1), dim3(256), 0, s, sa);
    hipLaunchKernelGGL(colsum_finish_kernel, dim3(cdiv(C, 256), 1), dim3(256), 0, s, partial, w.var + (size_t)m * C, C, nslab, (float)N,
                       (float)N, 0, (const float*)nullptr, (float*)nullptr);
  }
  HIP_TRY(hipGetLastError());
  return WCT_OK;
}

static int launch_slot_cov(const float* x, int N, int C, int m, int nsplit, int ksplit, float eps, const WctCarve& w, hipStream_t s) {
  const int BT = C >= 128 ? 128 : 64;
  const size_t cc = (size_t)C * C;
  CovArgs ca;
  ca.x[0] = ca.x[1] = x; ca.n[0] = ca.n[1] = N;
  ca.mean = w.mean + (size_t)m * C; ca.scale = w.scale + m; ca.partial = w.cov_partial + (size_t)m * w.nsplit * cc;
  ca.C = C; ca.ksplit = ksplit; ca.nsplit = nsplit; ca.ntile = cdiv(C, BT); ca.shared_style = 0;
  dim3 grid(ca.ntile * (ca.ntile + 1) / 2, nsplit, 1);
  if (BT == 128) hipLaunchKernelGGL((cov_f16x2_kernel<128>), grid, dim3(256), 0, s, ca);
  else hipLaunchKernelGGL((cov_f16x2_kernel<64>), grid, dim3(256), 0, s, ca);
  hipLaunchKernelGGL(cov_finish_kernel, dim3(cdiv(C, 64), cdiv(C, 64), 1), dim3(256), 0, s,
                     ca.partial, ca.scale, w.A + m * cc, C, nsplit, BT, 1.f / (float)(N - 1), 1.f / (float)(N - 1), eps, 0, w.A0 + m * cc);
  HIP_TRY(hipGetLastError());
  return WCT_OK;
}

int launch_plan_stats(const SlotPlan& sp, int C, bool with_var, bool with_cov, float eps, hipStream_t s) {
  int rc;
  for (int m = 0; m < 2 * sp.P; ++m) {
    const SlotPlan::Slot& t = sp.slot[m];
    if (!t.n) continue;
    if ((rc = launch_slot_means(t.x, t.n, C, m, t.lay.nslab, sp.w, with_var, s, m ? nullptr : sp.u0, m ? nullptr : sp.umax0))) return rc;
    if (with_cov && (rc = launch_slot_cov(t.x, t.n, C, m, t.lay.nsplit, t.lay.ksplit, eps, sp.w, s))) return rc;
  }
  return WCT_OK;
}
```

### wct_tf_amd/csrc/wct.hip

```cpp
#include "wct_stages.h"
#include "jacobi_dev.h"
#include <algorithm>
#include <type_traits>



template <int BC, int BP, typename Args = ApplyArgs>
__global__ __launch_bounds__(256, 2) void apply_f16x2_kernel(Args p) {
  constexpr bool SEGB = std::is_same<Args, ApplySegBatchArgs>::value;
  constexpr bool SEG = std::is_same<Args, ApplySegArgs>::value || SEGB;
  constexpr int TM = BC / 64, TN = BP / 64;
  constexpr int MI = BC * 4 / 256, XI = BP * 4 / 256;
  __shared__ __attribute__((aligned(16))) unsigned char lm[2][BC * 64];
  __shared__ __attribute__((aligned(16))) unsigned char lx[2][BP * 64];
  typedef unsigned int u32x4 __attribute__((ext_vector_type(4)));
  const int tid = threadIdx.x, lane = tid & 63, wave = tid >> 6;
  const int wm = wave >> 1, wn = wave & 1;
  const int pair = blockIdx.z;
  const int n0 = blockIdx.x * BP, c0 = blockIdx.y * BC;
  int seg0 = 0, N = p.N;
  [[maybe_unused]] int row0 = 0;
  if constexpr (SEGB) {
    const int f = seg_frame(p.fl[pair]), lab = seg_label(p.fl[pair]);
    const int first = p.seg_off[f * (WCT_MIX_MAX + 1) + lab];
    N = p.seg_off[f * (WCT_MIX_MAX + 1) + lab + 1] - first;
    if (n0 >= N) return;
    row0 = f * p.N;
    seg0 = row0 + first;
  } else if constexpr (SEG) {
    seg0 = p.seg_off[p.lab[pair]];
    N = p.seg_off[p.lab[pair] + 1] - seg0;
    if (n0 >= N) return;
  }
  const int C = p.C;
  const float* x = p.x + (SEG ? (size_t)seg0 * C : (size_t)pair * N * C);
  const float* M = p.M + (size_t)pair * C * C;
  const float* mean = p.mean + (size_t)pair * 2 * C;
  const float sx = p.xscale[2 * pair];
  float sM = 1.f;
  {
    const float m = __uint_as_float(p.mabs[pair]);
    if (m > 0.f) { int e; frexpf(m, &e); sM = ldexpf(1.f, 14 - e); }
  }

  const float* mp[MI]; const float* xp[XI];
  int moff[MI], xoff[XI], xk[XI];
#pragma unroll
  for (int i = 0; i < MI; ++i) {
    const int item = tid + i * 256, row = item >> 2, kq = item & 3;
    mp[i] = M + (size_t)min(c0 + row, C - 1) * C + kq * 8;
    moff[i] = (row * 4 + (kq ^ ((row >> 2) & 3))) * 16;
  }
#pragma unroll
  for (int i = 0; i < XI; ++i) {
    const int item = tid + i * 256, row = item >> 2, kq = item & 3;
    xp[i] = x + (size_t)min(n0 + row, N - 1) * C + kq * 8;
    xoff[i] = (row * 4 + (kq ^ ((row >> 2) & 3))) * 16;
    xk[i] = kq * 8;
  }

  f32x16 acc[TM][TN];
#pragma unroll
  for (int i = 0; i < TM; ++i)
#pragma unroll
    for (int j = 0; j < TN; ++j)
#pragma unroll
      for (int r = 0; r < 16; ++r) acc[i][j][r] = 0.f;

  f32x4 rm[MI][2], rx[XI][2];
  auto load = [&](int k0) {
#pragma unroll
    for (int i = 0; i < MI; ++i) {
      rm[i][0] = *reinterpret_cast<const f32x4*>(mp[i] + k0);
      rm[i][1] = *reinterpret_cast<const f32x4*>(mp[i] + k0 + 4);
    }
#pragma unroll
    for (int i = 0; i < XI; ++i) {
      rx[i][0] = *reinterpret_cast<const f32x4*>(xp[i] + k0) - *reinterpret_cast<const f32x4*>(mean + k0 + xk[i]);
      rx[i][1] = *reinterpret_cast<const f32x4*>(xp[i] + k0 + 4) - *reinterpret_cast<const f32x4*>(mean + k0 + xk[i] + 4);
    }
  };
  auto split_store = [&](const f32x4 (&r)[2], float sc, unsigned char* hi, unsigned char* lo, int off) {
    half8 h, l;
#pragma unroll
    for (int j = 0; j < 8; ++j) {
      const float v = r[j >> 2][j & 3] * sc;
      h[j] = (half_t)v;
      l[j] = (half_t)(v - (float)h[j]);
    }
    *reinterpret_cast<half8*>(hi + off) = h;
    *reinterpret_cast<half8*>(lo + off) = l;
  };

  load(0);
  for (int k0 = 0; k0 < C; k0 += 32) {
#pragma unroll
    for (int i = 0; i < MI; ++i) split_store(rm[i], sM, lm[0], lm[1], moff[i]);
#pragma unroll
    for (int i = 0; i < XI; ++i) split_store(rx[i], sx, lx[0], lx[1], xoff[i]);
    __syncthreads();
    if (k0 + 32 < C) load(k0 + 32);
#pragma unroll
    for (int ks = 0; ks < 2; ++ks) {
      const int chunk = ks * 2 + (lane >> 5);
      half8 ah[TM], al[TM], bh[TN], bl[TN];
#pragma unroll
      for (int i = 0; i < TM; ++i) {
        const int r = (wm * TM + i) * 32 + (lane & 31);
        const int off = (r * 4 + (chunk ^ ((r >> 2) & 3))) * 16;
        ah[i] = *reinterpret_cast<const half8*>(lm[0] + off);
        al[i] = *reinterpret_cast<const half8*>(lm[1] + off);
      }
#pragma unroll
      for (int j = 0; j < TN; ++j) {
        const int r = (wn * TN + j) * 32 + (lane & 31);
        const int off = (r * 4 + (chunk ^ ((r >> 2) & 3))) * 16;
        bh[j] = *reinterpret_cast<const half8*>(lx[0] + off);
        bl[j] = *reinterpret_cast<const half8*>(lx[1] + off);
      }
#pragma unroll
      for (int i = 0; i < TM; ++i)
#pragma unroll
        for (int j = 0; j < TN; ++j) {
          acc[i][j] = __builtin_amdgcn_mfma_f32_32x32x16_f16(al[i], bh[j], acc[i][j], 0, 0, 0);
          acc[i][j] = __builtin_amdgcn_mfma_f32_32x32x16_f16(ah[i], bl[j], acc[i][j], 0, 0, 0);
          acc[i][j] = __builtin_amdgcn_mfma_f32_32x32x16_f16(ah[i], bh[j], acc[i][j], 0, 0, 0);
        }
    }
    __syncthreads();
  }

  const float inv = 1.f / (sx * sM);
  const float* bias = p.bias + (size_t)pair * C;
  const int kgrp = lane >> 5;
  f32x4 bvs[TM][4];
#pragma unroll
  for (int i = 0; i < TM; ++i)
#pragma unroll
    for (int rq = 0; rq < 4; ++rq) {
      const int co = c0 + (wm * TM + i) * 32 + 8 * rq + 4 * kgrp;
      const f32x4 z = {0.f, 0.f, 0.f, 0.f};
      bvs[i][rq] = co < C ? *reinterpret_cast<const f32x4*>(bias + co) : z;
    }
  int dst[TN];
  if constexpr (SEG)
#pragma unroll
    for (int j = 0; j < TN; ++j) {
      const int n = n0 + (wn * TN + j) * 32 + (lane & 31);
      dst[j] = p.perm[seg0 + (n < N ? n : 0)];
      if constexpr (SEGB) dst[j] += row0;
    }
#pragma unroll
  for (int j = 0; j < TN; ++j) {
    const int n = n0 + (wn * TN + j) * 32 + (lane & 31);
    const bool n_ok = n < N;
    const size_t row = SEG ? (size_t)dst[j] * C : ((size_t)pair * N + (n_ok ? n : 0)) * C;
#pragma unroll
    for (int i = 0; i < TM; ++i) {
      const int cb = c0 + (wm * TM + i) * 32;
      unsigned pk[4][2];
#pragma unroll
      for (int rq = 0; rq < 4; ++rq) {
        const int co = cb + 8 * rq + 4 * kgrp;
        const f32x4 bv = bvs[i][rq];
        f32x4 v;
#pragma unroll
        for (int q = 0; q < 4; ++q) v[q] = acc[i][j][rq * 4 + q] * inv + bv[q];
        if (p.out32 && n_ok && co < C) *reinterpret_cast<f32x4*>(p.out32 + row + co) = v;
        typedef _Float16 h2 __attribute__((ext_vector_type(2)));
        h2 lo = {(half_t)v[0], (half_t)v[1]}, hi = {(half_t)v[2], (half_t)v[3]};
        pk[rq][0] = __builtin_bit_cast(unsigned, lo);
        pk[rq][1] = __builtin_bit_cast(unsigned, hi);
      }
      if (p.out16) {
#pragma unroll
        for (int m = 0; m < 2; ++m) {
          auto sxw = __builtin_amdgcn_permlane32_swap(pk[2 * m][0], pk[2 * m + 1][0], false, false);
          auto syw = __builtin_amdgcn_permlane32_swap(pk[2 * m][1], pk[2 * m + 1][1], false, false);
          u32x4 o = {sxw[0], syw[0], sxw[1], syw[1]};
          const int co = cb + 16 * m + 8 * kgrp;
          if (n_ok && co < C) *reinterpret_cast<u32x4*>(p.out16 + row + co) = o;
        }
      }
    }
  }
}

int launch_apply_seg(const ApplySegArgs& a, int nmax, int P, hipStream_t s) {
  const int C = a.C;
  if (C >= 128) hipLaunchKernelGGL((apply_f16x2_kernel<128, 128, ApplySegArgs>), dim3(cdiv(nmax, 128), cdiv(C, 128), P), dim3(256), 0, s, a);
  else hipLaunchKernelGGL((apply_f16x2_kernel<64, 128, ApplySegArgs>), dim3(cdiv(nmax, 128), cdiv(C, 64), P), dim3(256), 0, s, a);
  HIP_TRY(hipGetLastError());
  return WCT_OK;
}

int launch_apply_seg_batch(const ApplySegBatchArgs& a, int nmax, int P, hipStream_t s) {
  const int C = a.C;
  if (C >= 128) hipLaunchKernelGGL((apply_f16x2_kernel<128, 128, ApplySegBatchArgs>), dim3(cdiv(nmax, 128), cdiv(C, 128), P), dim3(256), 0, s, a);
  else hipLaunchKernelGGL((apply_f16x2_kernel<64, 128, ApplySegBatchArgs>), dim3(cdiv(nmax, 128), cdiv(C, 64), P), dim3(256), 0, s, a);
  HIP_TRY(hipGetLastError());
  return WCT_OK;
}

static int wct_nslab(int N) { int s = cdiv(N, 64); return s < 1 ? 1 : (s > 256 ? 256 : s); }

static void cov_split(int C, int Nmax, int P, int* nsplit, int* ksplit) {
  const int nt = C >= 128 ? cdiv(C, 128) : 1;
  const int tiles = nt * (nt + 1) / 2 * P;
  int want = 32 / tiles;
  if (want < 1) want = 1;
  int ks = cdiv(cdiv(Nmax, want), 32) * 32;
  if (ks < 256) ks = 256;
  *ksplit = ks;
  *nsplit = cdiv(Nmax, ks);
}

PairLayout pair_layout(int C, int Nc, int Ns) {
  PairLayout L;
  const int Nmax = Nc > Ns ? Nc : Ns;
  L.nslab = wct_nslab(Nmax);
  cov_split(C, Nmax, 1, &L.nsplit, &L.ksplit);
  return L;
}

WctCarve carve(void* base, int C, int P, const PairLayout& lay) {
  WctCarve w;
  w.nslab = lay.nslab; w.nsplit = lay.nsplit; w.ksplit = lay.ksplit;
  size_t off = 0;
  char* b = reinterpret_cast<char*>(base);
  auto take = [&](size_t bytes) { void* p = b ? b + off : nullptr; off += align_up(bytes); return p; };
  const size_t cc = (size_t)C * C * sizeof(float);
  w.mean = (float*)take((size_t)2 * P * C * sizeof(float));
  w.var = (float*)take((size_t)2 * P * C * sizeof(float));
  w.stat_partial = (float*)take((size_t)2 * P * w.nslab * C * sizeof(float));
  w.absmax = (float*)take((size_t)2 * P * w.nslab * sizeof(float));
  w.scale = (float*)take((size_t)2 * P * sizeof(float));
  w.cov_partial = (float*)take((size_t)2 * P * w.nsplit * cc);
  w.A = (float*)take(2 * P * cc);
  w.A0 = (float*)take(2 * P * cc);
  w.refresh = (int*)take((size_t)2 * P * sizeof(int));
  w.V = (float*)take(2 * P * cc);
  w.d = (float*)take((size_t)2 * P * C * sizeof(float));
  w.G = (float*)take(2 * P * cc);
  w.X = (float*)take(2 * P * cc);
  w.S2 = (float*)take(7 * P * cc);
  w.Tw = (float*)take(2 * P * cc);
  w.Tcs = w.Tw + (size_t)C * C;
  w.T = (float*)take(P * cc);
  w.M = (float*)take(P * cc);
  w.bias = (float*)take((size_t)P * C * sizeof(float));
  w.mabs = (unsigned*)take((size_t)P * sizeof(unsigned));
  w.jacobi_bytes = jacobi_workspace_bytes(C, 2 * P) + 4 * (1024 + 64 * sizeof(JacobiState));
  w.jacobi_ws = take(w.jacobi_bytes);
  w.mix = (float*)take((size_t)2 * C * sizeof(float));
  w.total = off;
  return w;
}

size_t wct_workspace_bytes(int C, int Nc, int Ns, int P) {
  const int Cw = C < 32 ? 32 : C;
  return carve(nullptr, Cw, P, pair_layout(Cw, Nc, Ns)).total;
}

int launch_blend(const WctCarve& w, int C, int P, float alpha, int shared_style, hipStream_t s) {
  const size_t cc = (size_t)C * C;
  GemmArgs g = {};
  g.A = w.Tcs; g.lda = C; g.a_kmajor = 0; g.B = w.Tw; g.ldb = C; g.b_kmajor = 1; g.sA = shared_style ? 0 : 2 * cc; g.sB = 2 * cc;
  g.M = C; g.N = C; g.K = C; g.ksplit = C; g.out32 = w.M; g.ldo = C; g.s_out = cc;
  g.blend = 1; g.alpha = alpha; g.mabs = w.mabs;
  return launch_gemm(g, 1, P, s);
}

static int launch_blend_apply(const WctCarve& w, const float* content, int Nc, int C, int P, float alpha, int shared_style,
                              half_t* out16, float* out32, hipStream_t s) {
  int rc;
  if ((rc = launch_blend(w, C, P, alpha, shared_style, s))) return rc;
  {
    ApplyArgs a;
    a.x = content; a.N = Nc; a.C = C; a.mean = w.mean; a.M = w.M; a.bias = w.bias;
    a.xscale = w.scale; a.mabs = w.mabs; a.out16 = out16; a.out32 = out32;
    if (C >= 128) hipLaunchKernelGGL((apply_f16x2_kernel<128, 128>), dim3(cdiv(Nc, 128), cdiv(C, 128), P), dim3(256), 0, s, a);
    else hipLaunchKernelGGL((apply_f16x2_kernel<64, 128>), dim3(cdiv(Nc, 128), cdiv(C, 64), P), dim3(256), 0, s, a);
  }
  HIP_TRY(hipGetLastError());
  return WCT_OK;
}

WctStyleKey wct_style_key(int C, int Nc, int Ns) {
  const PairLayout L = pair_layout(std::max(C, 32), Nc, Ns);
  return WctStyleKey{L.nslab, L.nsplit, L.ksplit};
}
size_t wct_style_state_floats(int C) { return (size_t)2 * C + (size_t)C * C; }

template <typename Ref>
__global__ __launch_bounds__(256) void style_load_kernel(Ref r, float* mean, float* var, float* Tw, int C, int with_T) {
  const int k = blockIdx.y;
  const float* src = r.state[k];
  const size_t cc = (size_t)C * C, n = (size_t)2 * C + (with_T ? cc : 0), slot = (size_t)(2 * k + 1);
  for (size_t i = (blockIdx.x * (size_t)blockDim.x + threadIdx.x) * 4; i < n; i += (size_t)gridDim.x * blockDim.x * 4) {
    const f32x4 v = *reinterpret_cast<const f32x4*>(src + i);
    float* dst = i < (size_t)C ? mean + slot * C + i : (i < (size_t)2 * C ? var + slot * C + (i - C) : Tw + slot * cc + (i - 2 * C));
    *reinterpret_cast<f32x4*>(dst) = v;
  }
}

static int launch_style_load(const WctStyleRef& r, int K, const WctCarve& w, int C, bool with_T, hipStream_t s) {
  for (int k = 0; k < K; ++k) ARG_CHECK(r.state[k] != nullptr);
  const size_t n4 = ((size_t)2 * C + (with_T ? (size_t)C * C : 0)) / 4;
  hipLaunchKernelGGL(style_load_kernel<WctStyleRef>, dim3((unsigned)std::min<size_t>((n4 + 255) / 256, 256), K), dim3(256), 0, s, r, w.mean,
                     w.var, w.Tw, C, with_T ? 1 : 0);
  HIP_TRY(hipGetLastError());
  return WCT_OK;
}

int launch_style_load_slots(const WctStyleSlots& r, int P, const WctCarve& w, int C, bool with_T, hipStream_t s) {
  ARG_CHECK(P >= 1 && P <= WCT_PLAN_PAIRS);
  for (int p = 0; p < P; ++p) ARG_CHECK(r.state[p] != nullptr);
  const size_t n4 = ((size_t)2 * C + (with_T ? (size_t)C * C : 0)) / 4;
  hipLaunchKernelGGL(style_load_kernel<WctStyleSlots>, dim3((unsigned)std::min<size_t>((n4 + 255) / 256, 256), P), dim3(256), 0, s, r, w.mean,
                     w.var, w.Tw, C, with_T ? 1 : 0);
  HIP_TRY(hipGetLastError());
  return WCT_OK;
}

static void style_plan(SlotPlan* sp, void* base, int C, const float* style, int Ns, const WctStyleKey& key) {
  *sp = SlotPlan{};
  sp->P = 1; sp->skip = WCT_SKIP_CONTENT; sp->nwhite = 0;
  sp->slot[1] = {style, Ns, PairLayout{key.nslab, key.nsplit, key.ksplit}};
  plan_carve(sp, base, C);
}

size_t wct_style_workspace_bytes(int C, int Ns, const WctStyleKey& key) {
  SlotPlan sp;
  style_plan(&sp, nullptr, C, nullptr, Ns, key);
  return sp.total;
}

int launch_style_state(const float* style, int Ns, int C, const WctStyleKey& key, int adain, int mode, float eps_in, void* workspace,
                       size_t workspace_bytes, int* eig_fail, hipStream_t s, float* state) {
  ARG_CHECK(style && state && C % 32 == 0 && C >= 32 && C <= 1024 && Ns >= (adain ? 1 : 2) && (size_t)Ns * C * 4 < ((size_t)1 << 31));
  ARG_CHECK(adain || mode == WCT_MODE_NP || mode == WCT_MODE_TF);
  ARG_CHECK(key.nslab >= 1 && key.nslab <= 256 && key.nsplit >= 1 && key.ksplit >= 256 && key.ksplit % 32 == 0 &&
            (long long)key.nsplit * key.ksplit >= Ns);
  SlotPlan sp;
  style_plan(&sp, workspace, C, style, Ns, key);
  ARG_CHECK(workspace_bytes >= sp.total);
  const WctCarve& w = sp.w;
  int rc;
  if (adain) {
    if ((rc = launch_plan_stats(sp, C, true, false, 0.f, s))) return rc;
    HIP_TRY(hipMemcpyAsync(state + C, w.var + C, (size_t)C * sizeof(float), hipMemcpyDeviceToDevice, s));
  } else {
    if ((rc = launch_plan_stats(sp, C, false, true, cov_eps(mode, eps_in), s))) return rc;
    if ((rc = launch_eig_stage(w, C, sp.P, sp.skip, 1, nullptr, eig_fail, s))) return rc;
    if ((rc = launch_spectral_tail(w, C, sp.P, 1.f, mode, eps_in, sp.skip, sp.nwhite, s))) return rc;
    HIP_TRY(hipMemcpyAsync(state + 2 * C, w.Tw + (size_t)C * C, (size_t)C * C * sizeof(float), hipMemcpyDeviceToDevice, s));
  }
  HIP_TRY(hipMemcpyAsync(state, w.mean + C, (size_t)C * sizeof(float), hipMemcpyDeviceToDevice, s));
  return WCT_OK;
}

int launch_wct(const float* content, int Nc, const float* style, int Ns, int C, int P, float alpha, int mode, float eps_in,
               half_t* out16, float* out32, void* workspace, size_t workspace_bytes, int* sweeps_dev,
               int stages, hipStream_t s, int shared_style, int* eig_fail, const WctFeatStats* stats, const WctStyleRef* prep,
               const WctWarmRef* warm) {
  ARG_CHECK(C % 32 == 0 && C >= 32 && C <= 1024 && Nc >= 2 && Ns >= 2 && P >= 1 && P <= 32);
  ARG_CHECK(!warm || (warm->basis && (shared_style == 0 || prep)));
  if (prep) shared_style = WCT_SKIP_STYLE;
  ARG_CHECK(mode == WCT_MODE_NP || mode == WCT_MODE_TF);
  ARG_CHECK((size_t)Nc * C * 4 < ((size_t)1 << 31) && (size_t)Ns * C * 4 < ((size_t)1 << 31));
  WctCarve w = carve(workspace, C, P, pair_layout(C, Nc, Ns));
  ARG_CHECK(workspace_bytes >= w.total);
  int rc;
  if (stages & WCT_STAGE_COV) {
    if ((rc = launch_means(content, Nc, style, Ns, C, P, w, false, shared_style, s, stats))) return rc;
    if ((rc = launch_cov(content, Nc, style, Ns, C, P, w, cov_eps(mode, eps_in), shared_style, s))) return rc;
  }
  if (stages & WCT_STAGE_EIG) {
    const bool rotate = warm && warm->valid;
    if (rotate && (rc = launch_warm_rotate(w, C, P, warm->basis, s))) return rc;
    if ((rc = launch_eig_stage(w, C, P, shared_style, (stages & WCT_STAGE_EIG_FP32UPDATE) ? 0 : 1, sweeps_dev, eig_fail, s, rotate ? 0 : 2)))
      return rc;
    if (rotate && (rc = launch_warm_compose(w, C, P, warm->basis, s))) return rc;
    if (warm && (rc = launch_warm_store(w.V + (size_t)2 * (P - 1) * C * C, w.X, warm->basis, C, s))) return rc;
  }
  if (!(stages & WCT_STAGE_APPLY)) return WCT_OK;

  if (prep && (rc = launch_style_load(*prep, 1, w, C, true, s))) return rc;
  if ((rc = launch_spectral_tail(w, C, P, alpha, mode, eps_in, shared_style, P, s))) return rc;
  return launch_blend_apply(w, content, Nc, C, P, alpha, shared_style, out16, out32, s);
}

void plan_carve(SlotPlan* sp, void* base, int C) {
  PairLayout mx = {1, 1, 0};
  for (int m = 0; m < 2 * sp->P; ++m)
    if (sp->slot[m].n) { mx.nslab = std::max(mx.nslab, sp->slot[m].lay.nslab); mx.nsplit = std::max(mx.nsplit, sp->slot[m].lay.nsplit); }
  sp->w = carve(base, C, std::max(sp->P, 1), mx);
  sp->total = sp->w.total;
}

bool plan_fits(const SlotPlan& sp, int C) {
  for (int m = 0; m < 2 * sp.P; ++m)
    if ((size_t)sp.slot[m].n * C * 4 >= ((size_t)1 << 31)) return false;
  return true;
}

static bool mix_plan(SlotPlan* sp, void* base, int C, const float* content, int Nc, const float* const* styles, const int* Ns,
                     int K, const float* lambda, int nmin, const WctFeatStats* stats, bool prepared = false) {
  if (!Ns || !lambda || K < 1 || K > WCT_MIX_MAX) return false;
  int ref = 0;
  for (int k = 0; k < K; ++k) {
    if ((styles && !styles[k]) || Ns[k] < nmin || !(lambda[k] >= 0.f && lambda[k] <= 1.f)) return false;
    if (lambda[k] > lambda[ref]) ref = k;
  }
  const int Cw = std::max(C, 32);
  *sp = SlotPlan{};
  sp->P = K; sp->skip = WCT_SKIP_MIX; sp->nwhite = 1;
  if (stats) { sp->u0 = stats->u[0]; sp->umax0 = stats->umax[0]; }
  sp->slot[0] = {content, Nc, pair_layout(Cw, Nc, Ns[ref])};
  for (int k = 0; k < K; ++k) sp->slot[2 * k + 1] = {styles ? styles[k] : nullptr, Ns[k], pair_layout(Cw, Nc, Ns[k])};
  if (prepared) {
    sp->skip = WCT_SKIP_MIX_STYLE;
    for (int k = 0; k < K; ++k) sp->slot[2 * k + 1].n = 0;
  }
  plan_carve(sp, base, Cw);
  return true;
}

size_t wct_mix_workspace_bytes(int C, int Nc, const int* Ns, int K, const float* lambda) {
  SlotPlan sp;
  return mix_plan(&sp, nullptr, C, nullptr, Nc, nullptr, Ns, K, lambda, 1, nullptr) ? sp.total : 0;
}

struct MixWeights { float lambda[WCT_MIX_MAX]; int K; };

__global__ __launch_bounds__(256) void wct_mix_kernel(float* Tw, float* bias, int C, MixWeights mw) {
  const size_t cc = (size_t)C * C, n4 = cc / 4;
  for (size_t i = blockIdx.x * (size_t)blockDim.x + threadIdx.x; i < n4; i += (size_t)gridDim.x * blockDim.x) {
    f32x4 acc = {0.f, 0.f, 0.f, 0.f};
    for (int k = 0; k < mw.K; ++k) {
      const f32x4 t = *reinterpret_cast<const f32x4*>(Tw + (2 * k + 1) * cc + i * 4);
#pragma unroll
      for (int j = 0; j < 4; ++j) acc[j] = fmaf(mw.lambda[k], t[j], acc[j]);
    }
    *reinterpret_cast<f32x4*>(Tw + cc + i * 4) = acc;
  }
  if (blockIdx.x == 0)
    for (int c = threadIdx.x; c < C; c += blockDim.x) {
      float acc = 0.f;
      for (int k = 0; k < mw.K; ++k) acc = fmaf(mw.lambda[k], bias[(size_t)k * C + c], acc);
      bias[c] = acc;
    }
}

int launch_wct_mix(const float* content, int Nc, const float* const* styles, const int* Ns, int K, const float* lambda, int C,
                   float alpha, int mode, float eps_in, half_t* out16, float* out32, void* workspace, size_t workspace_bytes,
                   int* sweeps_dev, int stages, hipStream_t s, int* eig_fail, const WctFeatStats* stats, const WctStyleRef* prep) {
  SlotPlan sp;
  ARG_CHECK(C % 32 == 0 && C >= 32 && C <= 1024 && Nc >= 2 && content && (styles || prep) &&
            mix_plan(&sp, workspace, C, content, Nc, prep ? nullptr : styles, Ns, K, lambda, 2, stats, prep != nullptr));
  ARG_CHECK(mode == WCT_MODE_NP || mode == WCT_MODE_TF);
  ARG_CHECK(plan_fits(sp, C));
  ARG_CHECK(workspace_bytes >= sp.total);
  const WctCarve& w = sp.w;
  int rc;
  if ((stages & WCT_STAGE_COV) && (rc = launch_plan_stats(sp, C, false, true, cov_eps(mode, eps_in), s))) return rc;
  if ((stages & WCT_STAGE_EIG) && (rc = launch_eig_stage(w, C, sp.P, sp.skip, 1, sweeps_dev, eig_fail, s))) return rc;
  if (!(stages & WCT_STAGE_APPLY)) return WCT_OK;
  if (prep && (rc = launch_style_load(*prep, K, w, C, true, s))) return rc;
  if ((rc = launch_spectral_tail(w, C, sp.P, alpha, mode, eps_in, sp.skip, sp.nwhite, s))) return rc;
  MixWeights mw = {};
  mw.K = K;
  for (int k = 0; k < K; ++k) mw.lambda[k] = lambda[k];
  const size_t n4 = (size_t)C * C / 4;
  hipLaunchKernelGGL(wct_mix_kernel, dim3((unsigned)std::min<size_t>((n4 + 255) / 256, 1024)), dim3(256), 0, s, w.Tw, w.bias, C, mw);
  HIP_TRY(hipGetLastError());
  return launch_blend_apply(w, content, Nc, C, 1, alpha, 0, out16, out32, s);
}

__global__ void adain_apply_kernel(const float* x, size_t n4_per_pair, int C, const float* mean, const float* var,
                                   float alpha, float eps, half_t* out16, float* out32, int shared_style,
                                   const float* mix_mu = nullptr, const float* mix_sd = nullptr) {
  const int pair = blockIdx.y;
  const int cq = C / 4;
  const float* mp = mean + (size_t)pair * 2 * C;
  const float* vp = var + (size_t)pair * 2 * C;
  const float* ms = mix_mu ? mix_mu : mean + (size_t)(shared_style ? 0 : pair) * 2 * C + C;
  const float* vs = var + (size_t)(shared_style ? 0 : pair) * 2 * C + C;
  const size_t base = (size_t)pair * n4_per_pair;
  for (size_t i = blockIdx.x * (size_t)blockDim.x + threadIdx.x; i < n4_per_pair; i += (size_t)gridDim.x * blockDim.x) {
    const int c = (int)(i % cq) * 4;
    f32x4 v = *reinterpret_cast<const f32x4*>(x + (base + i) * 4);
    f32x4 o;
#pragma unroll
    for (int j = 0; j < 4; ++j) {
      const float inv = 1.f / sqrtf(vp[c + j] + eps);
      const float sd = mix_sd ? mix_sd[c + j] : sqrtf(vs[c + j]);
      const float y = (v[j] - mp[c + j]) * inv * sd + ms[c + j];
      o[j] = alpha * y + (1.f - alpha) * v[j];
    }
    if (out32) *reinterpret_cast<f32x4*>(out32 + (base + i) * 4) = o;
    if (out16) {
      half4 h;
#pragma unroll
      for (int j = 0; j < 4; ++j) h[j] = (half_t)o[j];
      *reinterpret_cast<half4*>(out16 + (base + i) * 4) = h;
    }
  }
}

int launch_adain(const float* content, int Nc, const float* style, int Ns, int C, int P, float alpha, float eps,
                 half_t* out16, float* out32, void* workspace, size_t workspace_bytes, hipStream_t s, int shared_style,
                 const WctFeatStats* stats, const WctStyleRef* prep) {
  ARG_CHECK(C % 4 == 0 && C <= 1024 && Nc >= 1 && Ns >= 1 && P >= 1 && P <= 32);
  if (prep) shared_style = WCT_SKIP_STYLE;
  const int Cw = C < 32 ? 32 : C;
  WctCarve w = carve(workspace, Cw, P, pair_layout(Cw, Nc, Ns));
  ARG_CHECK(workspace_bytes >= w.total);
  int rc;
  if ((rc = launch_means(content, Nc, style, Ns, C, P, w, true, shared_style, s, stats))) return rc;
  if (prep && (rc = launch_style_load(*prep, 1, w, C, false, s))) return rc;
  const size_t n4 = (size_t)Nc * C / 4;
  hipLaunchKernelGGL(adain_apply_kernel, dim3(rows_grid(Nc, C), P), dim3(256), 0, s, content, n4, C, w.mean, w.var, alpha, eps, out16, out32, shared_style);
  HIP_TRY(hipGetLastError());
  return WCT_OK;
}

__global__ void adain_mix_moments_kernel(const float* mean, const float* var, float* mix, int C, MixWeights mw) {
  const int c = blockIdx.x * blockDim.x + threadIdx.x;
  if (c >= C) return;
  float mu = 0.f, sd = 0.f;
  for (int k = 0; k < mw.K; ++k) {
    mu = fmaf(mw.lambda[k], mean[(size_t)(2 * k + 1) * C + c], mu);
    sd = fmaf(mw.lambda[k], sqrtf(var[(size_t)(2 * k + 1) * C + c]), sd);
  }
  mix[c] = mu;
  mix[C + c] = sd;
}

int launch_adain_mix(const float* content, int Nc, const float* const* styles, const int* Ns, int K, const float* lambda, int C,
                     float alpha, float eps, half_t* out16, float* out32, void* workspace, size_t workspace_bytes, hipStream_t s,
                     const WctFeatStats* stats, const WctStyleRef* prep) {
  SlotPlan sp;
// ... 19 lines not shown
```

### wct_tf_amd/csrc/wct_stages.h

```cpp
#pragma once
#include "common.h"

constexpr int WCT_SKIP_MIX = 2;
constexpr int WCT_SKIP_STYLE = 3, WCT_SKIP_CONTENT = 4, WCT_SKIP_MIX_STYLE = 5;
constexpr int WCT_SKIP_STYLES = 6;
__device__ __host__ __forceinline__ bool skip_style_mat(int mat, int shared_style) {
  if (shared_style >= WCT_SKIP_STYLE)
    return shared_style == WCT_SKIP_STYLE ? (mat & 1) != 0
                                          : (shared_style == WCT_SKIP_CONTENT ? (mat & 1) == 0
                                                                              : (shared_style == WCT_SKIP_MIX_STYLE ? mat > 0 : (mat & 1) != 0));
  return shared_style == WCT_SKIP_MIX ? ((mat & 1) == 0 && mat > 0) : (shared_style && (mat & 1) && mat > 1);
}
__device__ __host__ __forceinline__ bool one_content(int shared_style) { return shared_style == WCT_SKIP_MIX || shared_style == WCT_SKIP_MIX_STYLE; }
__device__ __host__ __forceinline__ bool one_style(int shared_style) { return shared_style == 1 || shared_style == WCT_SKIP_STYLE; }

constexpr int EIG_CORRECT = 2;
constexpr float JACOBI_TOL_FN = 1.5e-2f;
constexpr float JACOBI_TOL_FN2 = 4e-2f;
constexpr float JACOBI_TOL_FN_WCT = EIG_CORRECT >= 2 ? JACOBI_TOL_FN2 : (EIG_CORRECT ? JACOBI_TOL_FN : 0.f);

static inline size_t align_up(size_t x) { return (x + 255) & ~(size_t)255; }

struct WctCarve {
  float *mean, *var, *stat_partial, *absmax, *scale, *cov_partial, *A, *A0, *V, *d, *G, *X, *S2, *Tw, *Tcs, *T, *M, *bias, *mix;
  unsigned* mabs; int* refresh;
  void* jacobi_ws; size_t jacobi_bytes;
  int nslab, nsplit, ksplit;
  size_t total;
};

struct PairLayout { int nslab, nsplit, ksplit; };
PairLayout pair_layout(int C, int Nc, int Ns);
WctCarve carve(void* base, int C, int P, const PairLayout& lay);

static inline float cov_eps(int mode, float eps_in) {
  return mode == WCT_MODE_TF ? (eps_in >= 0.f ? eps_in : 1e-8f) : 0.f;
}

static inline unsigned rows_grid(size_t N, int C) {
  const size_t blocks = (N * C / 4 + 255) / 256;
  return (unsigned)(blocks > 2048 ? 2048 : blocks);
}

constexpr int WCT_PLAN_PAIRS = 32;
struct SlotPlan {
  int P, skip, nwhite;
  struct Slot { const float* x; int n; PairLayout lay; } slot[2 * WCT_PLAN_PAIRS];
  const float* u0; const unsigned* umax0;
  WctCarve w;
  size_t total;
};
void plan_carve(SlotPlan* sp, void* base, int C);
bool plan_fits(const SlotPlan& sp, int C);

struct ApplyArgs {
  const float* x; int N; int C;
  const float* mean;
  const float* M; const float* bias;
  const float* xscale;
  const unsigned* mabs;
  half_t* out16; float* out32;
};
struct ApplySegArgs : ApplyArgs { const int* seg_off; const int* perm; int lab[WCT_MIX_MAX]; };
struct ApplySegBatchArgs : ApplyArgs { const int* seg_off; const int* perm; unsigned char fl[WCT_PLAN_PAIRS]; };
__device__ __host__ __forceinline__ int seg_frame(unsigned char fl) { return fl >> 3; }
__device__ __host__ __forceinline__ int seg_label(unsigned char fl) { return fl & 7; }

int launch_means(const float* content, int Nc, const float* style, int Ns, int C, int P, const WctCarve& w, bool with_var,
                 int shared_style, hipStream_t s, const WctFeatStats* fs = nullptr);
int launch_cov(const float* content, int Nc, const float* style, int Ns, int C, int P, const WctCarve& w, float eps, int shared_style,
               hipStream_t s);
int launch_plan_stats(const SlotPlan& sp, int C, bool with_var, bool with_cov, float eps, hipStream_t s);
int launch_eig_stage(const WctCarve& w, int C, int P, int skip, int u_f16, int* sweeps_dev, int* eig_fail, hipStream_t s,
                     int check_from = 2);
int launch_refresh(const WctCarve& w, int C, int P, int shared_style, hipStream_t s, bool always = false);
int launch_spectral_tail(const WctCarve& w, int C, int P, float alpha, int mode, float eps_in, int shared_style, int nwhite, hipStream_t s);
int launch_spectral_function(const float* A, const float* V, float* G, float* X, float* out, int C, int nbatch, size_t stride,
                             size_t out_stride, int kind, float shift, hipStream_t s, float* scratch2 = nullptr);
int launch_blend(const WctCarve& w, int C, int P, float alpha, int shared_style, hipStream_t s);
int launch_apply_seg(const ApplySegArgs& a, int nmax, int P, hipStream_t s);
int launch_apply_seg_batch(const ApplySegBatchArgs& a, int nmax, int P, hipStream_t s);
int launch_warm_rotate(const WctCarve& w, int C, int P, const float* V0, hipStream_t s);
int launch_warm_compose(const WctCarve& w, int C, int P, const float* V0, hipStream_t s);
int launch_warm_store(const float* V, float* scratch, float* basis, int C, hipStream_t s);
int launch_style_load_slots(const WctStyleSlots& r, int P, const WctCarve& w, int C, bool with_T, hipStream_t s);
```

Baseline: 670.3.

## Recompute level-1 relu1_1 features from the image inside cov and apply kernels

```diff
diff --git a/wct_tf_amd/csrc/api.hip b/wct_tf_amd/csrc/api.hip
--- a/wct_tf_amd/csrc/api.hip
+++ b/wct_tf_amd/csrc/api.hip
@@ -546,13 +546,14 @@
   half_t* cur = (half_t*)c->act[0].p;
   half_t* nxt = (half_t*)c->act[1].p;
   static const int fuse_conv1_env = getenv("WCT_FUSE_CONV1") ? atoi(getenv("WCT_FUSE_CONV1")) : 1;
-  const bool fuse_conv1 = fuse_conv1_env && deepest > 1 && !taps32[1];
+  const bool stats1 = usum && usum[1];
+  const bool fuse_conv1 = fuse_conv1_env && deepest > 1 && !taps32[1] && !stats1;
   if (!fuse_conv1) {
     ConvFirstArgs a;
     a.x = img; a.wfrag = c->first_w; a.bias = c->first_b;
     a.y16 = deepest > 1 ? cur : nullptr; a.y32 = taps32[1];
     a.B = B; a.H = H; a.W = W; a.clamp01 = clamp01;
-    a.usum = usum && taps32[1] ? usum[1] : nullptr; a.umax = a.usum ? umax[1] : nullptr;
+    a.usum = stats1 ? usum[1] : nullptr; a.umax = a.usum ? umax[1] : nullptr;
     const double px = (double)B * H * W;
     ProfScope ps(c, 1, 2.0 * px * 27 * 64, px * (12 + 64 * ((a.y16 ? 2 : 0) + (a.y32 ? 4 : 0))));
     TRY(launch_conv_first(a, c->stream));
@@ -642,8 +643,12 @@
                          const WctFeatStats* st = nullptr, const WctStyleRef* prep = nullptr ,
                          const WctWarmRef* warm = nullptr ) {
   const int shared = (flags & WCT_FLAG_STYLE_SHARED) ? 1 : 0;
-  const StageCost cost = {(double)P * 2.0 * C * C * ((double)Nc + Ns), (double)P * 2.0 * ((double)Nc + Ns) * C * 4,
-                          (double)P * (2.0 * C * C * Nc + 6.0 * C * C * C), (double)P * Nc * C * (4 + (out16 ? 2 : 0) + (out32 ? 4 : 0)),
+  const double rc = st && st->img[0] ? 12.0 : C * 4.0, rs = st && st->img[1] ? 12.0 : C * 4.0;
+  const double fl1 = 2.0 * 27 * 64;
+  const StageCost cost = {(double)P * 2.0 * C * C * ((double)Nc + Ns) + (double)P * fl1 * ((rc == 12.0 ? Nc : 0) + (rs == 12.0 ? Ns : 0)),
+                          (double)P * ((double)Nc * (rc + (rc == 12.0 ? C * 4.0 / 16 : C * 4.0)) + (double)Ns * (rs + (rs == 12.0 ? C * 4.0 / 16 : C * 4.0))),
+                          (double)P * (2.0 * C * C * Nc + 6.0 * C * C * C) + (rc == 12.0 ? (double)P * fl1 * Nc : 0.0),
+                          (double)P * Nc * (rc + C * ((out16 ? 2 : 0) + (out32 ? 4 : 0))),
                           (double)P * (2.0 * Nc + 2.0 * Ns) * C * 4 + (double)P * Nc * C * 6};
   return run_stages(c, wct_workspace_bytes(C, Nc, Ns, P), flags, cost, [&](int mode, int stages) {
     if (!stages) return launch_adain(fc, Nc, fs, Ns, C, P, alpha, 1e-5f, out16, out32, c->wct_ws.p, c->wct_ws.cap, c->stream, shared, st, prep);
@@ -1192,10 +1197,15 @@
   return on != 0;
 }
 
+static bool level1_from_image(unsigned flags, int W) {
+  static const int on = getenv("WCT_LEVEL1_FROM_IMAGE") ? atoi(getenv("WCT_LEVEL1_FROM_IMAGE")) : 1;
+  return on != 0 && fuse_stats() && !(flags & WCT_FLAG_ADAIN) && W % 32 == 0;
+}
+
 template <typename StyleAt, typename Transform>
 static int stylize_levels(wct_ctx* c, const float* img_c, const void* content_raw, int B, int Hc, int Wc, const int* levels,
                           int n_levels, unsigned flags, size_t umax_clear, int clear_from, StyleAt&& style_at,
-                          Transform&& transform, uint8_t* out) {
+                          Transform&& transform, uint8_t* out, bool plain_wct = false ) {
   unsigned* const umax_c = (unsigned*)c->umax.p;
   const float* cur = img_c;
   int H = Hc, W = Wc;
@@ -1203,9 +1213,12 @@
     const int l = levels[i], C = LEVEL_C[l];
     int h, w;
     level_dims(H, W, l, &h, &w);
-    TRY(ensure(c, c->feat_c, (size_t)B * h * w * C * 4));
+    const bool from_img = plain_wct && l == 1 && level1_from_image(flags, W);
     float* ctaps[6] = {nullptr, nullptr, nullptr, nullptr, nullptr, nullptr};
-    ctaps[l] = (float*)c->feat_c.p;
+    if (!from_img) {
+      TRY(ensure(c, c->feat_c, (size_t)B * h * w * C * 4));
+      ctaps[l] = (float*)c->feat_c.p;
+    }
     float* us_c[6] = {nullptr, nullptr, nullptr, nullptr, nullptr, nullptr};
     unsigned* um_c[6] = {nullptr, nullptr, nullptr, nullptr, nullptr, nullptr};
     if (fuse_stats() && w % 16 == 0) {
@@ -1215,6 +1228,7 @@
     }
     WctFeatStats st = {};
     st.u[0] = us_c[l]; st.umax[0] = um_c[l];
+    if (from_img) { st.img[0] = cur; st.ih[0] = H; st.iw[0] = W; st.clamp[0] = i > 0; st.w1frag = c->first_w; st.bias1 = c->first_b; }
     TRY(run_encoder(c, cur, B, H, W, i > 0, l, ctaps, us_c, um_c));
     TRY(ensure(c, c->wct_out, (size_t)B * h * w * C * 2));
     if (l == 5 && (flags & WCT_FLAG_SWAP5)) {
@@ -1262,6 +1276,7 @@
   TRY(ensure(c, c->umax, 7 * UROW * sizeof(unsigned)));
   unsigned* const umax_c = (unsigned*)c->umax.p;
   if (want_stats) HIP_TRY(hipMemsetAsync(c->umax.p, 0, 7 * UROW * sizeof(unsigned), c->stream));
+  const bool style_img = level1_from_image(flags, Ws);
   float* taps[6] = {nullptr, nullptr, nullptr, nullptr, nullptr, nullptr};
   float* us_s[6] = {nullptr, nullptr, nullptr, nullptr, nullptr, nullptr};
   unsigned* um_s[6] = {nullptr, nullptr, nullptr, nullptr, nullptr, nullptr};
@@ -1269,8 +1284,10 @@
     const int l = levels[i];
     int h, w;
     level_dims(Hs, Ws, l, &h, &w);
-    TRY(ensure(c, c->feat_s[l], (size_t)Bs * h * w * LEVEL_C[l] * 4));
-    taps[l] = (float*)c->feat_s[l].p;
+    if (!(l == 1 && style_img)) {
+      TRY(ensure(c, c->feat_s[l], (size_t)Bs * h * w * LEVEL_C[l] * 4));
+      taps[l] = (float*)c->feat_s[l].p;
+    }
     if (want_stats && w % 16 == 0) {
       TRY(ensure(c, c->usum_s[l], (size_t)Bs * h * (w / 16) * LEVEL_C[l] * 4));
       us_s[l] = (float*)c->usum_s[l].p; um_s[l] = umax_c + UROW * l;
@@ -1287,9 +1304,13 @@
                           int hs, ws;
                           const float* fs = style_at(l, 0, &hs, &ws);
                           st.u[1] = us_s[l]; st.umax[1] = um_s[l];
-                          return run_transform(c, (float*)c->feat_c.p, h * w, fs, hs * ws, C, B, alpha, flags, -1.f,
+                          if (l == 1 && style_img) {
+                            fs = nullptr;
+                            st.img[1] = img_s; st.ih[1] = Hs; st.iw[1] = Ws; st.clamp[1] = 0; st.w1frag = c->first_w; st.bias1 = c->first_b;
+                          }
+                          return run_transform(c, st.img[0] ? nullptr : (float*)c->feat_c.p, h * w, fs, hs * ws, C, B, alpha, flags, -1.f,
                                                (half_t*)c->wct_out.p, nullptr, nullptr, &st);
-                        }, out);
+                        }, out, true);
 }
 
 extern "C" int wct_stylize(wct_ctx* c, const uint8_t* content, int Hc, int Wc, const uint8_t* style, int Hs, int Ws,
diff --git a/wct_tf_amd/csrc/common.h b/wct_tf_amd/csrc/common.h
--- a/wct_tf_amd/csrc/common.h
+++ b/wct_tf_amd/csrc/common.h
@@ -142,7 +142,11 @@
 
 enum { WCT_MODE_NP = 0, WCT_MODE_TF = 1 };
 
-struct WctFeatStats { const float* u[2]; const unsigned* umax[2]; };
+struct WctFeatStats {
+  const float* u[2]; const unsigned* umax[2];
+  const float* img[2]; int ih[2], iw[2], clamp[2];
+  const half_t* w1frag; const float* bias1;
+};
 
 struct WctStyleKey { int nslab, nsplit, ksplit; };
 WctStyleKey wct_style_key(int C, int Nc, int Ns);
diff --git a/wct_tf_amd/csrc/conv.hip b/wct_tf_amd/csrc/conv.hip
--- a/wct_tf_amd/csrc/conv.hip
+++ b/wct_tf_amd/csrc/conv.hip
@@ -527,6 +527,7 @@
   __syncthreads();
   const unsigned char* pb = reinterpret_cast<const unsigned char*>(patch);
   unsigned char* const wt = tr[wave];
+  const bool stored = p.y32 || p.y16;
   float vmax = 0.f;
   for (int tile = 0; tile < CF_TILES; ++tile) {
   const int x0 = (sx * CF_TILES + tile) * 16;
@@ -566,7 +567,7 @@
 #pragma unroll
         for (int j = 0; j < 4; ++j) v[j] = fmaxf(acc[nt][rq * 4 + j] + bias[nt][rq][j], 0.f);
         const int piece = nt * 8 + 2 * rq + kgrp;
-        *reinterpret_cast<f32x4*>(wt + (px * 16 + (piece ^ (px & 15))) * 16) = v;
+        if (stored) *reinterpret_cast<f32x4*>(wt + (px * 16 + (piece ^ (px & 15))) * 16) = v;
         if (p.usum) {
           f32x4 t = v;
           unit_row_sum4(t);
@@ -619,7 +620,7 @@
 
 int launch_conv_first(const ConvFirstArgs& a, hipStream_t s) {
   ARG_CHECK(a.H > 1 && a.W > 1 && a.B > 0);
-  ARG_CHECK(!a.usum || (a.y32 && a.umax && a.W % 16 == 0));
+  ARG_CHECK(!a.usum || (a.umax && a.W % 16 == 0));
   const int strips_x = cdiv(a.W, 64), tiles_y = cdiv(a.H, 16);
   hipLaunchKernelGGL(conv_first_kernel, dim3(strips_x * tiles_y, a.B), dim3(256), 0, s, a, strips_x);
   HIP_TRY(hipGetLastError());
diff --git a/wct_tf_amd/csrc/stats_gemm.hip b/wct_tf_amd/csrc/stats_gemm.hip
--- a/wct_tf_amd/csrc/stats_gemm.hip
+++ b/wct_tf_amd/csrc/stats_gemm.hip
@@ -310,10 +310,12 @@
   float* partial;
   int C, ksplit, nsplit, ntile;
   int shared_style;
+  L1Side im[2];
+  const half_t* w1frag; const float* bias1;
 };
 
-template <int BT>
-__global__ __launch_bounds__(256, 2) void cov_f16x2_kernel(CovArgs p) {
+template <int BT, bool IMG = false>
+__global__ __launch_bounds__(256, IMG ? 4 : 2) void cov_f16x2_kernel(CovArgs p) {
   constexpr int TM = BT / 64;
   constexpr int KPT = BT * 32 / 256;
   constexpr int NPC = KPT / 8;
@@ -401,8 +403,113 @@
     }
   };
 
+  bool from_image = false;
+  if constexpr (IMG) {
+    static_assert(!IMG || BT == 64, "level 1 from the image: 64 channels");
+    const L1Side im = p.im[side];
+    if (im.img) {
+      from_image = true;
+      __shared__ unsigned patch[2 * L1_STRIDE];
+      const float* ib = im.img + (size_t)pair * im.H * im.W * 3;
+      const int nt = wave & 1, half = wave >> 1, kgrp = lane >> 5, odd = lane & 1;
+      half8 wh[2], wl[2];
+#pragma unroll
+      for (int ks = 0; ks < 2; ++ks) {
+        wh[ks] = *reinterpret_cast<const half8*>(p.w1frag + (((nt * 2 + ks) * 2 + 0) * 64 + lane) * 8);
+        wl[ks] = *reinterpret_cast<const half8*>(p.w1frag + (((nt * 2 + ks) * 2 + 1) * 64 + lane) * 8);
+      }
+      f32x4 b1[4], mu[4];
+#pragma unroll
+      for (int rq = 0; rq < 4; ++rq) {
+        b1[rq] = *reinterpret_cast<const f32x4*>(p.bias1 + nt * 32 + 8 * rq + 4 * kgrp);
+        mu[rq] = *reinterpret_cast<const f32x4*>(p.mean + mat * C + nt * 32 + 8 * rq + 4 * kgrp);
+      }
+      const L1Frag off = l1_frag_bases(lane);
+      if (tid < 2 * (L1_STRIDE - L1_WORDS)) patch[(tid / (L1_STRIDE - L1_WORDS)) * L1_STRIDE + L1_WORDS + tid % (L1_STRIDE - L1_WORDS)] = 0u;
+      const int kb = lane & 30;
+      int dst[4];
+#pragma unroll
+      for (int rq = 0; rq < 4; ++rq) {
+        const int ch = nt * 32 + 8 * rq + 4 * kgrp + odd;
+        dst[rq] = (ch * 4 + ((kb >> 3) ^ ((2 * rq + kgrp) & 3))) * 16 + (kb & 7) * 2;
+      }
+      const unsigned sel = odd ? 0x03020706u : 0x05040100u;
+      typedef float f32x2 __attribute__((ext_vector_type(2)));
+      typedef _Float16 h2 __attribute__((ext_vector_type(2)));
+      constexpr int SLOTS = (2 * L1_WORDS + 255) / 256;
+      int ty[2], tx[2];
+#pragma unroll
+      for (int t = 0; t < 2; ++t) { const int n = kbeg + 32 * t; ty[t] = n / im.W; tx[t] = n - ty[t] * im.W; }
+      float pre[SLOTS];
+      auto fetch = [&]() {
+#pragma unroll
+        for (int i = 0; i < SLOTS; ++i) {
+          const int e = min(tid + i * 256, 2 * L1_WORDS - 1), t = e >= L1_WORDS ? 1 : 0;
+          pre[i] = ib[l1_src(e - t * L1_WORDS, t ? ty[1] : ty[0], t ? tx[1] : tx[0], im.H, im.W)];
+        }
+      };
+      auto park = [&]() {
+#pragma unroll
+        for (int i = 0; i < SLOTS; ++i) {
+          const int e = tid + i * 256, t = e >= L1_WORDS ? 1 : 0;
+          if (e < 2 * L1_WORDS) patch[t * L1_STRIDE + e - t * L1_WORDS] = l1_pack(pre[i], im.clamp01);
+        }
+      };
+      auto mma_diag = [&](const unsigned char* hi, const unsigned char* lo) {
+#pragma unroll
+        for (int ks = 0; ks < 2; ++ks) {
+          const int chunk = ks * 2 + (lane >> 5);
+          const int ra_ = wm * 32 + (lane & 31), rb_ = wn * 32 + (lane & 31);
+          const int oa = (ra_ * 4 + (chunk ^ ((ra_ >> 2) & 3))) * 16, ob = (rb_ * 4 + (chunk ^ ((rb_ >> 2) & 3))) * 16;
+          const half8 ah = *reinterpret_cast<const half8*>(hi + oa), al = *reinterpret_cast<const half8*>(lo + oa);
+          const half8 bh = *reinterpret_cast<const half8*>(hi + ob), bl = *reinterpret_cast<const half8*>(lo + ob);
+          acc[0][0] = __builtin_amdgcn_mfma_f32_32x32x16_f16(al, bh, acc[0][0], 0, 0, 0);
+          acc[0][0] = __builtin_amdgcn_mfma_f32_32x32x16_f16(ah, bl, acc[0][0], 0, 0, 0);
+          acc[0][0] = __builtin_amdgcn_mfma_f32_32x32x16_f16(ah, bh, acc[0][0], 0, 0, 0);
+        }
+      };
+      if (kbeg < kend) fetch();
+      for (int k0 = kbeg; k0 < kend; k0 += 64) {
+        const bool two = k0 + 32 < kend;
+        park();
+        __syncthreads();
+#pragma unroll
+        for (int t = 0; t < 2; ++t) {
+          tx[t] += 64;
+          if (tx[t] >= im.W) { tx[t] -= im.W; ++ty[t]; }
+          if (tx[t] >= im.W) { tx[t] -= im.W; ++ty[t]; }
+        }
+        if (k0 + 64 < kend) fetch();
+        if (half == 0 || two) {
+          const f32x16 a1 = l1_tile(patch + half * L1_STRIDE, off, wh, wl);
+          unsigned char* const hi = lds[2 * half], * const lo = lds[2 * half + 1];
+#pragma unroll
+          for (int rq = 0; rq < 4; ++rq) {
+#pragma unroll
+            for (int jj = 0; jj < 2; ++jj) {
+              const f32x2 a2 = {a1[rq * 4 + 2 * jj], a1[rq * 4 + 2 * jj + 1]}, b2 = {b1[rq][2 * jj], b1[rq][2 * jj + 1]};
+              const f32x2 m2 = {mu[rq][2 * jj], mu[rq][2 * jj + 1]}, z2 = {0.f, 0.f}, s2 = {sc, sc};
+              const f32x2 r = __builtin_elementwise_max(a2 + b2, z2);
+              const f32x2 v = (r - m2) * s2;
+              const h2 hh = __builtin_convertvector(v, h2);
+              const h2 ll = __builtin_convertvector(v - __builtin_convertvector(hh, f32x2), h2);
+              const unsigned ph = __builtin_bit_cast(unsigned, hh), pl = __builtin_bit_cast(unsigned, ll);
+              const unsigned qh = (unsigned)__builtin_amdgcn_update_dpp(0, (int)ph, 0xB1, 0xF, 0xF, true);
+              const unsigned ql = (unsigned)__builtin_amdgcn_update_dpp(0, (int)pl, 0xB1, 0xF, 0xF, true);
+              *reinterpret_cast<unsigned*>(hi + dst[rq] + jj * 128) = __builtin_amdgcn_perm(qh, ph, sel);
+              *reinterpret_cast<unsigned*>(lo + dst[rq] + jj * 128) = __builtin_amdgcn_perm(ql, pl, sel);
+            }
+          }
+        }
+        __syncthreads();
+        mma_diag(lds[0], lds[1]);
+        if (two) mma_diag(lds[2], lds[3]);
+      }
+    }
+  }
   float ra[KPT], rb[KPT];
-  if (diag) {
+  if (from_image) {
+  } else if (diag) {
     if (kbeg < kend) load(ra, voff_a, kbeg);
     for (int k0 = kbeg; k0 < kend; k0 += 32) {
       if (k0 + 32 <= kend) split_store(ra, mean_a, k0, false, lds[0], lds[1]);
@@ -509,7 +616,7 @@
 }
 
 int launch_cov(const float* content, int Nc, const float* style, int Ns, int C, int P, const WctCarve& w, float eps, int shared_style,
-               hipStream_t s) {
+               hipStream_t s, const WctFeatStats* fs) {
   const int BT = C >= 128 ? 128 : 64;
   {
     CovArgs ca;
@@ -517,7 +624,19 @@
     ca.mean = w.mean; ca.scale = w.scale; ca.partial = w.cov_partial;
     ca.C = C; ca.ksplit = w.ksplit; ca.nsplit = w.nsplit; ca.ntile = cdiv(C, BT); ca.shared_style = shared_style;
     dim3 grid(ca.ntile * (ca.ntile + 1) / 2, w.nsplit, 2 * P);
-    if (BT == 128) hipLaunchKernelGGL((cov_f16x2_kernel<128>), grid, dim3(256), 0, s, ca);
+    bool from_image = false;
+    for (int b = 0; b < 2; ++b) {
+      ca.im[b] = L1Side{nullptr, 0, 0, 0};
+      if (fs && fs->img[b]) {
+        const int N = b ? Ns : Nc;
+        ARG_CHECK(C == 64 && fs->w1frag && fs->bias1 && fs->iw[b] % 32 == 0 && fs->ih[b] * fs->iw[b] == N && w.ksplit % 32 == 0);
+        ca.im[b] = L1Side{fs->img[b], fs->ih[b], fs->iw[b], fs->clamp[b]};
+        from_image = true;
+      }
+    }
+    ca.w1frag = fs ? fs->w1frag : nullptr; ca.bias1 = fs ? fs->bias1 : nullptr;
+    if (from_image) hipLaunchKernelGGL((cov_f16x2_kernel<64, true>), grid, dim3(256), 0, s, ca);
+    else if (BT == 128) hipLaunchKernelGGL((cov_f16x2_kernel<128>), grid, dim3(256), 0, s, ca);
     else hipLaunchKernelGGL((cov_f16x2_kernel<64>), grid, dim3(256), 0, s, ca);
     HIP_TRY(hipGetLastError());
   }
@@ -555,6 +674,7 @@
   ca.x[0] = ca.x[1] = x; ca.n[0] = ca.n[1] = N;
   ca.mean = w.mean + (size_t)m * C; ca.scale = w.scale + m; ca.partial = w.cov_partial + (size_t)m * w.nsplit * cc;
   ca.C = C; ca.ksplit = ksplit; ca.nsplit = nsplit; ca.ntile = cdiv(C, BT); ca.shared_style = 0;
+  ca.im[0] = ca.im[1] = L1Side{nullptr, 0, 0, 0}; ca.w1frag = nullptr; ca.bias1 = nullptr;
   dim3 grid(ca.ntile * (ca.ntile + 1) / 2, nsplit, 1);
   if (BT == 128) hipLaunchKernelGGL((cov_f16x2_kernel<128>), grid, dim3(256), 0, s, ca);
   else hipLaunchKernelGGL((cov_f16x2_kernel<64>), grid, dim3(256), 0, s, ca);
diff --git a/wct_tf_amd/csrc/wct.hip b/wct_tf_amd/csrc/wct.hip
--- a/wct_tf_amd/csrc/wct.hip
+++ b/wct_tf_amd/csrc/wct.hip
@@ -9,10 +9,12 @@
 __global__ __launch_bounds__(256, 2) void apply_f16x2_kernel(Args p) {
   constexpr bool SEGB = std::is_same<Args, ApplySegBatchArgs>::value;
   constexpr bool SEG = std::is_same<Args, ApplySegArgs>::value || SEGB;
+  constexpr bool IMG = std::is_same<Args, ApplyImgArgs>::value;
+  static_assert(!IMG || (BC == 64 && BP == 128), "level 1 from the image: 64 channels x 128 pixels");
   constexpr int TM = BC / 64, TN = BP / 64;
   constexpr int MI = BC * 4 / 256, XI = BP * 4 / 256;
   __shared__ __attribute__((aligned(16))) unsigned char lm[2][BC * 64];
-  __shared__ __attribute__((aligned(16))) unsigned char lx[2][BP * 64];
+  __shared__ __attribute__((aligned(16))) unsigned char lx[IMG ? 4 : 2][BP * 64];
   typedef unsigned int u32x4 __attribute__((ext_vector_type(4)));
   const int tid = threadIdx.x, lane = tid & 63, wave = tid >> 6;
   const int wm = wave >> 1, wn = wave & 1;
@@ -74,6 +76,7 @@
       rm[i][0] = *reinterpret_cast<const f32x4*>(mp[i] + k0);
       rm[i][1] = *reinterpret_cast<const f32x4*>(mp[i] + k0 + 4);
     }
+    if constexpr (!IMG)
 #pragma unroll
     for (int i = 0; i < XI; ++i) {
       rx[i][0] = *reinterpret_cast<const f32x4*>(xp[i] + k0) - *reinterpret_cast<const f32x4*>(mean + k0 + xk[i]);
@@ -93,12 +96,82 @@
   };
 
   load(0);
+  if constexpr (IMG) {
+    __shared__ unsigned patch[4 * L1_STRIDE];
+    const L1Side im = p.im;
+    const float* ib = im.img + (size_t)pair * im.H * im.W * 3;
+    constexpr int SLOTS = (4 * L1_WORDS + 255) / 256;
+    int ty[4], tx[4];
+    ty[0] = n0 / im.W; tx[0] = n0 - ty[0] * im.W;
+#pragma unroll
+    for (int t = 1; t < 4; ++t) {
+      const bool wrap = tx[t - 1] + 32 >= im.W;
+      ty[t] = wrap ? ty[t - 1] + 1 : ty[t - 1]; tx[t] = wrap ? 0 : tx[t - 1] + 32;
+    }
+#pragma unroll
+    for (int t = 1; t < 4; ++t)
+      if (n0 + 32 * t >= N) { ty[t] = im.H - 1; tx[t] = im.W - 32; }
+    float pre[SLOTS];
+#pragma unroll
+    for (int i = 0; i < SLOTS; ++i) {
+      const int e = min(tid + i * 256, 4 * L1_WORDS - 1), t = e / L1_WORDS;
+      const int y = t == 0 ? ty[0] : (t == 1 ? ty[1] : (t == 2 ? ty[2] : ty[3])), x0 = t == 0 ? tx[0] : (t == 1 ? tx[1] : (t == 2 ? tx[2] : tx[3]));
+      pre[i] = ib[l1_src(e - t * L1_WORDS, y, x0, im.H, im.W)];
+    }
+    const int nt = wave & 1, kgrp = lane >> 5;
+    half8 wh[2], wl[2];
+#pragma unroll
+    for (int ks = 0; ks < 2; ++ks) {
+      wh[ks] = *reinterpret_cast<const half8*>(p.w1frag + (((nt * 2 + ks) * 2 + 0) * 64 + lane) * 8);
+      wl[ks] = *reinterpret_cast<const half8*>(p.w1frag + (((nt * 2 + ks) * 2 + 1) * 64 + lane) * 8);
+    }
+    f32x4 b1[4], mu[4];
+#pragma unroll
+    for (int rq = 0; rq < 4; ++rq) {
+      b1[rq] = *reinterpret_cast<const f32x4*>(p.bias1 + nt * 32 + 8 * rq + 4 * kgrp);
+      mu[rq] = *reinterpret_cast<const f32x4*>(mean + nt * 32 + 8 * rq + 4 * kgrp);
+    }
+    const L1Frag off = l1_frag_bases(lane);
+    if (tid < 4 * (L1_STRIDE - L1_WORDS)) patch[(tid / (L1_STRIDE - L1_WORDS)) * L1_STRIDE + L1_WORDS + tid % (L1_STRIDE - L1_WORDS)] = 0u;
+#pragma unroll
+    for (int i = 0; i < SLOTS; ++i) {
+      const int e = tid + i * 256, t = e / L1_WORDS;
+      if (e < 4 * L1_WORDS) patch[t * L1_STRIDE + e - t * L1_WORDS] = l1_pack(pre[i], im.clamp01);
+    }
+    __syncthreads();
+#pragma unroll
+    for (int tt = 0; tt < 2; ++tt) {
+      const int t = (wave >> 1) * 2 + tt, row = t * 32 + (lane & 31);
+      const f32x16 a1 = l1_tile(patch + t * L1_STRIDE, off, wh, wl);
+#pragma unroll
+      for (int rq = 0; rq < 4; ++rq) {
+        typedef float f32x2 __attribute__((ext_vector_type(2)));
+        typedef _Float16 h2 __attribute__((ext_vector_type(2)));
+        h2 h[2], l[2];
+#pragma unroll
+        for (int jj = 0; jj < 2; ++jj) {
+          const f32x2 a2 = {a1[rq * 4 + 2 * jj], a1[rq * 4 + 2 * jj + 1]}, b2 = {b1[rq][2 * jj], b1[rq][2 * jj + 1]};
+          const f32x2 m2 = {mu[rq][2 * jj], mu[rq][2 * jj + 1]}, z2 = {0.f, 0.f}, s2 = {sx, sx};
+          const f32x2 r = __builtin_elementwise_max(a2 + b2, z2);
+          const f32x2 v = (r - m2) * s2;
+          h[jj] = __builtin_convertvector(v, h2);
+          l[jj] = __builtin_convertvector(v - __builtin_convertvector(h[jj], f32x2), h2);
+        }
+        typedef unsigned u32x2 __attribute__((ext_vector_type(2)));
+        const int o = (row * 4 + (rq ^ ((row >> 2) & 3))) * 16 + kgrp * 8;
+        *reinterpret_cast<u32x2*>(lx[2 * nt] + o) = u32x2{__builtin_bit_cast(unsigned, h[0]), __builtin_bit_cast(unsigned, h[1])};
+        *reinterpret_cast<u32x2*>(lx[2 * nt + 1] + o) = u32x2{__builtin_bit_cast(unsigned, l[0]), __builtin_bit_cast(unsigned, l[1])};
+      }
+    }
+  }
   for (int k0 = 0; k0 < C; k0 += 32) {
 #pragma unroll
     for (int i = 0; i < MI; ++i) split_store(rm[i], sM, lm[0], lm[1], moff[i]);
+    if constexpr (!IMG)
 #pragma unroll
     for (int i = 0; i < XI; ++i) split_store(rx[i], sx, lx[0], lx[1], xoff[i]);
     __syncthreads();
+    const unsigned char* const xh = lx[IMG ? (k0 >> 5) * 2 : 0], * const xl = lx[IMG ? (k0 >> 5) * 2 + 1 : 1];
     if (k0 + 32 < C) load(k0 + 32);
 #pragma unroll
     for (int ks = 0; ks < 2; ++ks) {
@@ -115,8 +188,8 @@
       for (int j = 0; j < TN; ++j) {
         const int r = (wn * TN + j) * 32 + (lane & 31);
         const int off = (r * 4 + (chunk ^ ((r >> 2) & 3))) * 16;
-        bh[j] = *reinterpret_cast<const half8*>(lx[0] + off);
-        bl[j] = *reinterpret_cast<const half8*>(lx[1] + off);
+        bh[j] = *reinterpret_cast<const half8*>(xh + off);
+        bl[j] = *reinterpret_cast<const half8*>(xl + off);
       }
 #pragma unroll
       for (int i = 0; i < TM; ++i)
@@ -272,15 +345,19 @@
 }
 
 static int launch_blend_apply(const WctCarve& w, const float* content, int Nc, int C, int P, float alpha, int shared_style,
-                              half_t* out16, float* out32, hipStream_t s) {
+                              half_t* out16, float* out32, hipStream_t s, const WctFeatStats* fs = nullptr) {
   int rc;
   if ((rc = launch_blend(w, C, P, alpha, shared_style, s))) return rc;
   {
-    ApplyArgs a;
+    ApplyImgArgs a;
     a.x = content; a.N = Nc; a.C = C; a.mean = w.mean; a.M = w.M; a.bias = w.bias;
     a.xscale = w.scale; a.mabs = w.mabs; a.out16 = out16; a.out32 = out32;
-    if (C >= 128) hipLaunchKernelGGL((apply_f16x2_kernel<128, 128>), dim3(cdiv(Nc, 128), cdiv(C, 128), P), dim3(256), 0, s, a);
-    else hipLaunchKernelGGL((apply_f16x2_kernel<64, 128>), dim3(cdiv(Nc, 128), cdiv(C, 64), P), dim3(256), 0, s, a);
+    if (fs && fs->img[0]) {
+      ARG_CHECK(C == 64 && fs->w1frag && fs->bias1 && fs->iw[0] % 32 == 0 && fs->ih[0] * fs->iw[0] == Nc);
+      a.im = L1Side{fs->img[0], fs->ih[0], fs->iw[0], fs->clamp[0]}; a.w1frag = fs->w1frag; a.bias1 = fs->bias1;
+      hipLaunchKernelGGL((apply_f16x2_kernel<64, 128, ApplyImgArgs>), dim3(cdiv(Nc, 128), 1, P), dim3(256), 0, s, a);
+    } else if (C >= 128) hipLaunchKernelGGL((apply_f16x2_kernel<128, 128>), dim3(cdiv(Nc, 128), cdiv(C, 128), P), dim3(256), 0, s, (const ApplyArgs&)a);
+    else hipLaunchKernelGGL((apply_f16x2_kernel<64, 128>), dim3(cdiv(Nc, 128), cdiv(C, 64), P), dim3(256), 0, s, (const ApplyArgs&)a);
   }
   HIP_TRY(hipGetLastError());
   return WCT_OK;
@@ -366,6 +443,8 @@
                const WctWarmRef* warm) {
   ARG_CHECK(C % 32 == 0 && C >= 32 && C <= 1024 && Nc >= 2 && Ns >= 2 && P >= 1 && P <= 32);
   ARG_CHECK(!warm || (warm->basis && (shared_style == 0 || prep)));
+  for (int b = 0; b < 2; ++b) ARG_CHECK((b ? style : content) || prep || (stats && stats->img[b] && stats->u[b] && stats->umax[b]));
+  ARG_CHECK(!(stats && (stats->img[0] || stats->img[1])) || (!prep && !warm));
   if (prep) shared_style = WCT_SKIP_STYLE;
   ARG_CHECK(mode == WCT_MODE_NP || mode == WCT_MODE_TF);
   ARG_CHECK((size_t)Nc * C * 4 < ((size_t)1 << 31) && (size_t)Ns * C * 4 < ((size_t)1 << 31));
@@ -374,7 +453,7 @@
   int rc;
   if (stages & WCT_STAGE_COV) {
     if ((rc = launch_means(content, Nc, style, Ns, C, P, w, false, shared_style, s, stats))) return rc;
-    if ((rc = launch_cov(content, Nc, style, Ns, C, P, w, cov_eps(mode, eps_in), shared_style, s))) return rc;
+    if ((rc = launch_cov(content, Nc, style, Ns, C, P, w, cov_eps(mode, eps_in), shared_style, s, stats))) return rc;
   }
   if (stages & WCT_STAGE_EIG) {
     const bool rotate = warm && warm->valid;
@@ -388,7 +467,7 @@
 
   if (prep && (rc = launch_style_load(*prep, 1, w, C, true, s))) return rc;
   if ((rc = launch_spectral_tail(w, C, P, alpha, mode, eps_in, shared_style, P, s))) return rc;
-  return launch_blend_apply(w, content, Nc, C, P, alpha, shared_style, out16, out32, s);
+  return launch_blend_apply(w, content, Nc, C, P, alpha, shared_style, out16, out32, s, stats);
 }
 
 void plan_carve(SlotPlan* sp, void* base, int C) {
diff --git a/wct_tf_amd/csrc/wct_stages.h b/wct_tf_amd/csrc/wct_stages.h
--- a/wct_tf_amd/csrc/wct_stages.h
+++ b/wct_tf_amd/csrc/wct_stages.h
@@ -66,10 +66,65 @@
 __device__ __host__ __forceinline__ int seg_frame(unsigned char fl) { return fl >> 3; }
 __device__ __host__ __forceinline__ int seg_label(unsigned char fl) { return fl & 7; }
 
+struct L1Side { const float* img; int H, W, clamp01; };
+constexpr int L1_PW = 34, L1_ROW = L1_PW * 3, L1_WORDS = 3 * L1_ROW;
+constexpr int L1_STRIDE = 320;
+
+#ifdef __HIPCC__
+__device__ __forceinline__ int l1_reflect(int i, int n) {
+  if (i < 0) i = -i;
+  if (i >= n) i = 2 * n - 2 - i;
+  i = i < 0 ? 0 : i;
+  return i >= n ? n - 1 : i;
+}
+__device__ __forceinline__ unsigned l1_pack(float raw, int clamp01) {
+  const float v = clamp01 ? fminf(fmaxf(raw, 0.f), 1.f) : raw;
+  const half_t hi = (half_t)v, lo = (half_t)(v - (float)hi);
+  return (unsigned)__builtin_bit_cast(unsigned short, hi) | ((unsigned)__builtin_bit_cast(unsigned short, lo) << 16);
+}
+__device__ __forceinline__ int l1_src(int e, int y, int x0, int H, int W) {
+  const int ky = e / L1_ROW, q = e - ky * L1_ROW, px = q / 3, c = q - px * 3;
+  return (l1_reflect(y - 1 + ky, H) * W + l1_reflect(x0 - 1 + px, W)) * 3 + c;
+}
+struct L1Frag { int b8, bR, bz; };
+__device__ __forceinline__ L1Frag l1_frag_bases(int lane) {
+  const int kgrp = lane >> 5, base = (lane & 31) * 3;
+  return L1Frag{base + kgrp * 8, base + kgrp * (L1_ROW - 1), kgrp ? L1_WORDS - (2 * L1_ROW + 1) : base};
+}
+__device__ __forceinline__ f32x16 l1_tile(const unsigned* patch, const L1Frag& f, const half8 (&wh)[2], const half8 (&wl)[2]) {
+  constexpr int R = L1_ROW;
+  typedef unsigned int u32x4 __attribute__((ext_vector_type(4)));
+  f32x16 a;
+#pragma unroll
+  for (int r = 0; r < 16; ++r) a[r] = 0.f;
+#pragma unroll
+  for (int ks = 0; ks < 2; ++ks) {
+    unsigned w[8], uh[4], ul[4];
+#pragma unroll
+    for (int j = 0; j < 8; ++j)
+      w[j] = ks == 0 ? (j == 0 ? patch[f.b8] : patch[f.bR + j])
+                     : (j < 2 ? patch[f.bR + R + 7 + j] : (j == 2 ? patch[f.b8 + 2 * R] : patch[f.bz + 2 * R + j - 2]));
+#pragma unroll
+    for (int i = 0; i < 4; ++i) {
+      uh[i] = __builtin_amdgcn_perm(w[2 * i + 1], w[2 * i], 0x05040100u);
+      ul[i] = __builtin_amdgcn_perm(w[2 * i + 1], w[2 * i], 0x07060302u);
+    }
+    const half8 bh = __builtin_bit_cast(half8, u32x4{uh[0], uh[1], uh[2], uh[3]});
+    const half8 bl = __builtin_bit_cast(half8, u32x4{ul[0], ul[1], ul[2], ul[3]});
+    a = __builtin_amdgcn_mfma_f32_32x32x16_f16(wl[ks], bh, a, 0, 0, 0);
+    a = __builtin_amdgcn_mfma_f32_32x32x16_f16(wh[ks], bl, a, 0, 0, 0);
+    a = __builtin_amdgcn_mfma_f32_32x32x16_f16(wh[ks], bh, a, 0, 0, 0);
+  }
+  return a;
+}
+#endif
+
+struct ApplyImgArgs : ApplyArgs { L1Side im; const half_t* w1frag; const float* bias1; };
+
 int launch_means(const float* content, int Nc, const float* style, int Ns, int C, int P, const WctCarve& w, bool with_var,
                  int shared_style, hipStream_t s, const WctFeatStats* fs = nullptr);
 int launch_cov(const float* content, int Nc, const float* style, int Ns, int C, int P, const WctCarve& w, float eps, int shared_style,
-               hipStream_t s);
+               hipStream_t s, const WctFeatStats* fs = nullptr);
 int launch_plan_stats(const SlotPlan& sp, int C, bool with_var, bool with_cov, float eps, hipStream_t s);
 int launch_eig_stage(const WctCarve& w, int C, int P, int skip, int u_f16, int* sweeps_dev, int* eig_fail, hipStream_t s,
                      int check_from = 2);
```

Result: no change. 675.6, median of 6 (+0.8%).
